# facebookresearch/seamless_communication

Hardware: AMD Instinct MI355X
Metric: S2ST utterances/sec (and real-time factor), seamlessM4T_v2_large, 10 s audio (higher is better)
Workload: dtype f32 activations x f16 weights, f32 accumulate

## Files before the change

### include/seamless_hip_internal.h

```cpp
#ifndef SEAMLESS_HIP_INTERNAL_H_
#define SEAMLESS_HIP_INTERNAL_H_

#include "seamless_hip.h"

#ifdef __cplusplus
extern "C" {
#endif

int sc_decoder_step_family(sc_model* m, int rows, int caller);

int sc_op_knob(const char* name, int dflt);

int sc_op_force_general_gemm(int on);
int32_t sc_op_voc_pack_plan(const int32_t* h_need, int32_t n, int64_t budget_rows, int32_t* h_group_first, int32_t cap);
int32_t sc_op_voc_tile_first(const int32_t* h_off, int32_t n, int32_t mul, int32_t tile_rows, int32_t* h_first);
int32_t sc_op_last_vocoder_packed_groups(sc_model* m);
int sc_op_single_plane(int on);
int sc_op_layernorm(const float* d_x, const float* d_gamma, const float* d_beta, float* d_y, int32_t rows, int32_t C,
                    int32_t act);
int sc_op_linear(const float* d_x, const void* d_w_f16, const float* d_bias, const float* d_res, float* d_y,
                 int32_t M, int32_t N, int32_t K, int32_t act, float alpha, int32_t split, int32_t force_gemv);
int sc_op_skinny_linear(const float* d_x, const void* d_w_f16, const float* d_bias, const float* d_res, float* d_y,
                        int32_t M, int32_t N, int32_t K, int32_t act, float alpha);
int sc_op_skinny_res_ln(const float* d_in, const void* d_w_f16, const float* d_bias, float* d_x_inout,
                        const float* d_gamma, const float* d_beta, float* d_h, int32_t M, int32_t N, int32_t K,
                        int32_t splits);
int sc_op_skinny_argmax(const float* d_x, const void* d_w_f16, int32_t M, int32_t N, int32_t K, int32_t step,
                        int32_t min_step_for_eos, int32_t force_eos_step, int32_t pad_idx, int32_t eos_idx,
                        int32_t unk_idx, float unk_penalty, int32_t* d_idx, float* d_lprob);

int sc_op_dstep_res_ln(const float* d_in, const void* d_w_f16, const float* d_bias, float* d_x_inout, const float* d_gamma,
                       const float* d_beta, float* d_h, int32_t M, int32_t N, int32_t K, int32_t splits);
int sc_op_dstep_linear_planes(const float* d_x, const void* d_w_f16, const float* d_bias, float* d_y, int32_t M, int32_t N, int32_t K,
                              int32_t act);
int sc_op_dstep_argmax(const float* d_x, const void* d_w_f16, int32_t M, int32_t N, int32_t K, int32_t step,
                       int32_t min_step_for_eos, int32_t force_eos_step, int32_t pad_idx, int32_t eos_idx, int32_t unk_idx,
                       float unk_penalty, int32_t ntl, int32_t* d_idx, float* d_lprob);
int sc_op_dstep_attention(const float* d_proj, int32_t S, const float* d_bias, float* d_kcache, float* d_vcache, int32_t cap,
                          int32_t pos, const int32_t* d_lens, int32_t cross, int32_t nb, int32_t heads, float* d_out);
int sc_op_dstep3_gemv(int32_t mode, const float* d_x, const void* d_w_f16, const float* d_bias, const float* d_gamma,
                      const float* d_beta, const float* d_res, float* d_y, float* d_h, int32_t M, int32_t N, int32_t K, int32_t act,
                      int32_t rg, int32_t shape);
int sc_op_dstep3_argmax(const float* d_x, const void* d_w_f16, int32_t M, int32_t N, int32_t K, int32_t step,
                        int32_t min_step_for_eos, int32_t force_eos_step, int32_t pad_idx, int32_t eos_idx, int32_t unk_idx,
                        float unk_penalty, int32_t* d_idx, float* d_lprob);
int sc_op_chain_bench(int32_t kind, int32_t rows, int32_t n, int32_t reps, float* us_per_kernel);
int sc_op_conv1d(const float* d_x, const void* d_w_f16_packed, const float* d_bias, const float* d_res, float* d_y,
                 int32_t nb, int32_t t_in, int32_t cin, int32_t cout, int32_t k, int32_t stride, int32_t pad,
                 int32_t dil, const int32_t* d_in_lens, int32_t in_act, int32_t act);
int sc_op_pack_conv_weight(const void* d_w_f16, void* d_dst_f16, int32_t cout, int32_t cin, int32_t k);
int sc_op_conv_transpose1d(const float* d_x, const void* d_v_f16, const void* d_g_f16, const float* d_bias,
                           float* d_y, int32_t nb, int32_t t_in, int32_t cin, int32_t cout, int32_t k,
                           int32_t stride, int32_t pad, int32_t in_act);
int sc_op_linear_presplit(const float* d_x, const void* d_w_f16, const float* d_bias, const float* d_res, float* d_y,
                          void* d_yh_f16, void* d_yl_f16, int32_t M, int32_t N, int32_t K, int32_t act, float alpha);
int sc_op_linear_presplit_argmax(const float* d_x, const void* d_w_f16, const float* d_bias, int32_t* d_idx, int32_t M, int32_t N,
                                 int32_t K);
int sc_op_conv1d_presplit(const float* d_x, const void* d_w_f16_packed, const float* d_bias, const float* d_res, float* d_y,
                          void* d_yh_f16, void* d_yl_f16, int32_t nb, int32_t t, int32_t cin, int32_t cout, int32_t k, int32_t pad,
                          int32_t dil, const unsigned char* d_row_valid, int32_t act);
int sc_op_resblock_pair_ps(const float* d_x, const void* d_w1_packed, const float* d_b1, const void* d_w2_packed, const float* d_b2,
                           float* d_out, int32_t nb, int32_t T, int32_t C, int32_t k, int32_t dil);
int sc_op_resblock_pair(const float* d_x, const void* d_w1_packed, const float* d_b1, const void* d_w2_packed,
                        const float* d_b2, float* d_out, int32_t nb, int32_t T, int32_t C, int32_t k, int32_t dil,
                        float slope, const float* d_avg_a, const float* d_avg_b);
int sc_op_mrf_fused(const float* d_x, const void* const* d_w1_packed, const float* const* d_b1, const void* const* d_w2_packed,
                    const float* const* d_b2, float* d_out, int32_t nb, int32_t T, int32_t C, const int32_t* k, const int32_t* dil,
                    float slope);
int sc_op_attention(const float* d_q, const float* d_k, const float* d_v, float* d_out, int32_t nb, int32_t heads,
                    int32_t sq, int32_t skv, int64_t ldq, int64_t ldk, int64_t ldv, int64_t ldo,
                    const int32_t* d_kv_lens, int32_t causal, const float* d_rel_k, int32_t rel_left,
                    int32_t rel_right);
int sc_op_attention_ex(const float* d_q, const float* d_k, const float* d_v, float* d_out, int32_t nb, int32_t heads,
                       int32_t sq, int32_t skv, int64_t ldq, int64_t ldk, int64_t ldv, int64_t ldo,
                       const int32_t* d_kv_lens, int32_t causal, const float* d_rel_k, int32_t rel_left,
                       int32_t rel_right, const int32_t* d_row_off, const float* d_rp_table, int64_t rp_ld,
                       const float* d_q_bias_u, const float* d_q_bias_v, void* d_out_hi, void* d_out_lo, int64_t ldoh);
int sc_op_glu_dwconv(const float* d_x, const float* d_w, float* d_y, int32_t nb, int32_t T, int32_t C, int32_t k,
                     const int32_t* d_lens);
int sc_op_glu_dwconv_ln(const float* d_x, const float* d_w, const float* d_gamma, const float* d_beta, int32_t act, void* d_yh_f16,
                        void* d_yl_f16, int32_t nb, int32_t T, int32_t C, int32_t k, const int32_t* d_lens, int32_t fused);
int sc_op_layernorm2(const float* d_x, const float* d_ga, const float* d_ba, const float* d_gb, const float* d_bb, float* d_y,
                     void* d_yh_f16, void* d_yl_f16, int32_t rows, int32_t C, int32_t fused);
int sc_op_argmax(const float* d_logits, int32_t rows, int32_t V, int32_t* d_idx, float* d_lprob);

int sc_op_beam_candidates(float* d_logits, int64_t ld, int32_t n_utt, int32_t beams, int32_t V, const float* d_cum, int32_t first_step,
                          int32_t no_eos, int32_t force_eos, int32_t pad_idx, int32_t eos_idx, int32_t unk_idx, float unk_penalty, int32_t K,
                          float* d_cand_val, int32_t* d_cand_idx, const int32_t* d_seqs, int32_t seq_ld, int32_t S, int32_t G,
                          const int32_t* d_rows, const int32_t* d_slots, int32_t chunked);
int sc_op_beam_candidates_banned(float* d_logits, int64_t ld, int32_t n_utt, int32_t beams, int32_t V, const float* d_cum,
                                 int32_t first_step, int32_t no_eos, int32_t force_eos, int32_t pad_idx, int32_t eos_idx, int32_t unk_idx,
                                 float unk_penalty, int32_t K, float* d_cand_val, int32_t* d_cand_idx, const int32_t* d_seqs,
                                 int32_t seq_ld, int32_t S, int32_t G, const int32_t* d_rows, const int32_t* d_slots, int32_t chunked,
                                 const int32_t* d_banned_tokens, const int32_t* d_banned_offsets, int32_t n_banned);
int sc_op_beam_select(const float* d_cand_val, const int32_t* d_cand_idx, const int32_t* d_seqs_cur, int32_t* d_seqs_new, float* d_fin_score,
                      int32_t* d_fin_len, int32_t* d_fin_seq, int32_t* d_fin_count, int32_t* d_done, int32_t* d_remaining, int32_t* d_tok,
                      int32_t* d_src_row, float* d_cum, int32_t* d_anc, int32_t anc_ld, const int32_t* d_slot_utt, const int32_t* d_slots,
                      int32_t n, int32_t beams, int32_t K, int32_t V, int32_t max_len, int32_t step, int32_t eos_idx, int32_t pad_idx,
                      int32_t normalize, float len_penalty);
int sc_op_beam_compact(const int32_t* d_done, int32_t* d_slot_utt, int32_t* d_slots, int32_t* d_rows, int32_t* d_seqs, float* d_cum,
                       int32_t* d_tok, int32_t* d_enc_lens, int32_t* d_anc, int32_t n, int32_t beams, int32_t max_len, int32_t anc_ld,
                       int32_t seq_len, int32_t anc_len);
int sc_op_gather_cache(const float* d_src, float* d_dst, const int32_t* d_src_row, int32_t rows, int32_t len, int32_t cap, int32_t M,
                       int32_t layers, int64_t layer_stride);
int sc_op_row_token_lprob(const float* d_logits, int64_t ld, int32_t rows, int32_t V, int32_t row_stride, int32_t token, float* d_out);

int sc_op_dstep_attention_ex(const float* d_proj, int32_t S, const float* d_bias, float* d_kcache, float* d_vcache, int32_t cap,
                             int32_t cache_rows, int32_t pos, const int32_t* d_lens, int32_t cross, int32_t nb, int32_t heads,
                             const int32_t* d_slot_rp, const int32_t* d_slot_lane, const int32_t* d_anc, const int32_t* d_kv_item,
                             int32_t kv_row_div, const int32_t* d_rows, float* d_out);
int sc_op_engine_step_close(const float* d_x, const void* d_w_f16, int32_t M, int32_t N, int32_t K, int32_t min_step_for_eos, int32_t pad_idx,
                            int32_t eos_idx, int32_t unk_idx, float unk_penalty, int32_t* d_slot_rp, const int32_t* d_rows, int32_t n_states,
                            int32_t cap, int32_t* d_tok, int32_t* d_pos, int32_t* d_finished, int32_t* d_out_len, const int32_t* d_limit,
                            const int32_t* d_prefix_len, float* d_score, int32_t* d_hist);
int sc_op_engine_admit(const int32_t* d_recs, int32_t n, int32_t n_states, int32_t cap, int32_t pad_idx, int32_t* d_tok, int32_t* d_pos,
                       int32_t* d_finished, int32_t* d_out_len, int32_t* d_limit, int32_t* d_prefix_len, int32_t* d_enc_lens, float* d_score,
                       int32_t* d_hist);
int sc_op_engine_set_slots(const int32_t* d_rids, int32_t n_live, int32_t slots, int32_t n_states, int32_t* d_slot_rp, int32_t* d_slot_lane,
                           const int32_t* d_pos, int32_t* d_rows);
int sc_op_engine_retire(const int32_t* h_rid, const int32_t* h_dst_rows, float* const* h_dst, int32_t n, int32_t n_states, int32_t cap, int32_t M,
                        const int32_t* d_out_len, const float* d_score, const int32_t* d_hist, const float* d_hidden, int32_t* d_stage);
int sc_op_dstep3_embed_ex(const int32_t* d_tok, const void* d_embed_f16, float scale, const float* d_pos_table, int32_t pos,
                          const int32_t* d_slot_rp, const int32_t* d_rows, int32_t rows, int32_t C, int32_t n_states, int32_t n_pos, int32_t vocab,
                          float* d_x);
int sc_op_dstep3_reduce_capture_ex(const float* d_partial, int32_t S, const float* d_bias, float* d_x_inout, const float* d_gamma, const float* d_beta,
                                   float* d_h, float* d_hrow, int64_t hrow_bs, int32_t hrow_rows, int32_t pos, const int32_t* d_slot_rp,
                                   const int32_t* d_rows, int32_t rows, int32_t C, int32_t n_states);
int sc_op_step_update(int32_t* d_next_tok, int32_t* d_hist, int32_t hist_ld, int32_t* d_finished, int32_t* d_out_len, const float* d_lprob,
                      float* d_score, int32_t nb, int32_t pos, int32_t pad_idx, int32_t eos_idx, int32_t* d_n_unfinished);
int sc_op_row_swap(float* d_k, float* d_v, float* d_cross, int32_t layers, int32_t pairs, const int32_t* h_src, const int32_t* h_dst, int32_t n_rows,
                   int32_t M, int32_t cap, int32_t s_enc, int32_t filled, int32_t* d_tok, int32_t* d_finished, int32_t* d_out_len,
                   int32_t* d_enc_lens, float* d_lprob, float* d_score, int32_t* d_hist, float* d_hidden);
int sc_op_align_lprob(const float* d_text, const float* d_feat, int32_t n, int32_t s_text, int32_t s_feat, int32_t C,
                      const int32_t* h_text_lens, const int32_t* h_feat_lens, float temperature, float* d_lprob);
int sc_op_mas(const float* d_lprob, int32_t n, int32_t s_text, int32_t s_feat, const int32_t* h_text_lens, const int32_t* h_feat_lens,
              int32_t* h_durations);
int sc_op_attention_hd(const float* d_q, const float* d_k, const float* d_v, float* d_out, int32_t nb, int32_t heads, int32_t sq, int32_t skv,
                       int64_t ldq, int64_t ldk, int64_t ldv, int64_t ldo, const int32_t* d_kv_lens, int32_t head_dim);
int sc_op_w2v2_frontend(const float* d_wav, int64_t wav_stride, const int32_t* h_num_samples, int32_t nb, const float* d_w, const float* d_bias,
                        const float* d_gamma, const float* d_beta, int32_t C, int32_t k, int32_t stride, float* d_out, int32_t t_rows,
                        float* d_stats);
int sc_op_w2v2_pos_conv(const float* d_x, const float* d_w, const float* d_bias, float* d_y, int32_t nb, int32_t T, int32_t C, int32_t groups,
                        int32_t k, const int32_t* d_lens);
int sc_op_kmeans(const float* d_x, const float* d_centroids, int32_t rows, int32_t C, int32_t K, int32_t* d_idx);

int sc_op_ecapa_chain(const float* d_x, const void* d_w_f16, const float* d_bias, const float* d_gamma, const float* d_beta, float* d_out, int32_t nb,
                      int32_t T, int32_t chunk, int32_t scale, int32_t dil);
int32_t sc_op_ecapa_chain_tile(int32_t chunk, int32_t scale, int32_t dil);
int sc_op_ecapa_relu_ln(const float* d_x, const float* d_item_bias, int32_t t_per_item, const float* d_gamma, const float* d_beta, float* d_y,
                        int32_t rows, int32_t C, int32_t act);
int sc_op_ecapa_se_gate(const float* d_x, int32_t nb, int32_t T, const int32_t* h_lens, int32_t C, int32_t S, const void* d_w1_f16, const float* d_b1,
                        const void* d_w2_f16, const float* d_b2, float* d_gate);
int sc_op_ecapa_pool(const float* d_x, const float* d_logits, int32_t nb, int32_t T, int32_t C, const int32_t* h_lens, float* d_pooled, float* d_gstats);
int sc_op_ecapa_tail(const float* d_pooled, int32_t nb, int32_t C2, const float* d_gamma, const float* d_beta, const void* d_w_f16, const float* d_bias,
                     int32_t E, float* d_out);
int32_t sc_op_prosody_last_launches(sc_prosody_encoder* p);

#ifdef __cplusplus
}
#endif
#endif
```

### seamless_communication_amd/_lib.py

```python
from __future__ import annotations

import ctypes as C
from pathlib import Path
from typing import Optional

import os

_VARIANT = os.environ.get("SC_LIB_VARIANT", "")
LIB_PATH = Path(__file__).resolve().parent / (f"libseamless_hip.{_VARIANT}.so" if _VARIANT else "libseamless_hip.so")

SC_ABI_VERSION = 10
SC_MAX_UPSAMPLES = 8
SC_MAX_RESBLOCK_KERNELS = 4
SC_MAX_RESBLOCK_DILATIONS = 4
SC_F16, SC_F32, SC_I32 = 0, 1, 2


class SeamlessHipError(RuntimeError):
    pass


class sc_tensor_desc(C.Structure):
    _fields_ = [
        ("name", C.c_char_p),
# ... 93 lines not shown
    "sc_abi_version": (C.c_int, []),
    "sc_load": (_P, [C.POINTER(sc_tensor_desc), C.c_size_t, C.POINTER(sc_config), C.c_int]),
    "sc_fork": (_P, [_P]),
    "sc_free": (None, [_P]),
    "sc_synchronize": (C.c_int, [_P]),
    "sc_wait_stream": (C.c_int, [_P, _P]),
    "sc_decoder_step_family": (C.c_int, [_P, C.c_int, C.c_int]),
    "sc_set_nar_tables": (C.c_int, [_P, _i, _P, _P, _P, _P, _P]),
    "sc_fbank": (C.c_int, [_P, _P, _i, C.c_int64, _P, _i, _P, _i, _P]),
    "sc_fbank_rate": (C.c_int, [_P, _P, _i, C.c_int64, _P, _i, _i, _P, _i, _P]),
    "sc_fbank_frames": (_i, [C.c_int64, _i]),
    "sc_encoder_out_len": (_i, [_P, _i]),
    "sc_encode_speech": (C.c_int, [_P, _P, _i, _i, _P, _P, _P]),
    "sc_encode_text": (C.c_int, [_P, _P, C.c_int32, C.c_int32, _P, _P]),
    "sc_mma_begin": (C.c_int, [_P, _P, C.c_int32, C.c_int32]),
    "sc_mma_step": (C.c_int, [_P, _P, C.c_int32, _P, C.c_int32, _P, _P, _P]),
    "sc_text_max_len": (_i, [_P, C.POINTER(sc_gen_opts), _i]),
    "sc_generate_text": (C.c_int, [_P, _P, _i, _i, _P, C.POINTER(sc_gen_opts), _P, _i, _P, _P, _P, _P]),
    "sc_generate_text_banned": (C.c_int, [_P, _P, _i, _i, _P, C.POINTER(sc_gen_opts), _P, _i, _P, _P, _P, _P, _P, _P, _i]),
    "sc_generate_text_capture": (C.c_int, [_P, _P, _i, _i, _P, C.POINTER(sc_gen_opts), _P, _i, _P, _P, _P, _P, _P, _P]),
    "sc_decode_text": (C.c_int, [_P, _P, _i, _i, _P, _P, _i, _P]),
    "sc_engine_create": (_P, [_P, C.POINTER(sc_engine_opts)]),
    "sc_engine_free": (None, [_P]),
    "sc_engine_attach": (C.c_int, [_P, _P]),
    "sc_engine_expect": (C.c_int, [_P, _i]),
    "sc_engine_get_stats": (C.c_int, [_P, C.POINTER(sc_engine_stats), _i]),
    "sc_t2u_nar": (C.c_int, [_P, _P, _i, _i, _P, _P, C.c_float, _P, _PI, _PI]),
    "sc_get_units": (C.c_int, [_P, _P]),
    "sc_get_durations": (C.c_int, [_P, _P, _P, _P]),
    "sc_vocoder_hop": (_i, [_P]),
    "sc_vocode": (C.c_int, [_P, _P, _i, _i, _P, _P, _P]),
    "sc_vocode_ragged": (C.c_int, [_P, _P, _i, _i, _P, _P, _P, _P]),
    "sc_vocoder_durations": (C.c_int, [_P, _P, _i, _i, _P]),
    "sc_t2u_ar": (C.c_int, [_P, _P, _i, _i, _P, C.POINTER(sc_gen_opts), _P, _i, _P, _i, _P, _P]),
    "sc_t2u_ar_max_len": (_i, [_P, C.POINTER(sc_gen_opts), _i]),
    "sc_last_padding": (C.c_int, [_P, _P, _P, _P]),
    "sc_s2st": (C.c_int, [_P, _P, _i, _i, _P, C.POINTER(sc_gen_opts), _P, _i, C.c_float, _P, _P, _P, _i, _P, _P, _i, _P, _P, _P]),
    "sc_prof_enable": (C.c_int, [C.c_int]),
    "sc_prof_reset": (C.c_int, []),
    "sc_prof_report": (C.c_int64, [C.c_char_p, C.c_int64]),
    "sc_text_to_char_seqs": (C.c_int32, [C.c_int32, _P, _P, _P, _P, _P, C.c_int32, C.c_int32, C.c_int32, _P, C.c_int32, C.c_int32,
                                         _P, _P, C.c_int32, _P]),
    "sc_ngram_blocked_tokens": (C.c_int32, [_PI, C.c_int32, C.c_int32, _PI, C.c_int32]),
    "sc_banned_blocked_tokens": (C.c_int32, [_PI, C.c_int32, _PI, _PI, C.c_int32, _PI, C.c_int32]),
    "sc_aligner_load": (_P, [C.POINTER(sc_tensor_desc), C.c_size_t, C.POINTER(sc_aligner_config), C.c_int]),
    "sc_aligner_free": (None, [_P]),
    "sc_align": (C.c_int, [_P, _P, _i, _i, _P, _P, _i, _P, _P, _P]),
    "sc_op_align_lprob": (C.c_int, [_P, _P, _i, _i, _i, _i, _P, _P, C.c_float, _P]),
    "sc_op_mas": (C.c_int, [_P, _i, _i, _i, _P, _P, _P]),
    "sc_unit_extractor_load": (_P, [C.POINTER(sc_tensor_desc), C.c_size_t, C.POINTER(sc_unit_extractor_config), C.c_int]),
    "sc_unit_extractor_free": (None, [_P]),
    "sc_unit_extractor_num_frames": (C.c_int32, [C.POINTER(sc_unit_extractor_config), C.c_int64]),
    "sc_extract_units": (C.c_int, [_P, _P, _i, C.c_int64, _P, _i, _P, _i, _P, _P]),
    "sc_op_attention_hd": (C.c_int, [_P, _P, _P, _P, _i, _i, _i, _i, C.c_int64, C.c_int64, C.c_int64, C.c_int64, _P, _i]),
    "sc_op_w2v2_frontend": (C.c_int, [_P, C.c_int64, _P, _i, _P, _P, _P, _P, _i, _i, _i, _P, _i, _P]),
    "sc_op_w2v2_pos_conv": (C.c_int, [_P, _P, _P, _P, _i, _i, _i, _i, _i, _P]),
    "sc_op_kmeans": (C.c_int, [_P, _P, _i, _i, _i, _P]),
    "sc_prosody_encoder_load": (_P, [C.POINTER(sc_tensor_desc), C.c_size_t, C.POINTER(sc_prosody_encoder_config), C.c_int]),
    "sc_prosody_encoder_free": (None, [_P]),
    "sc_prosody_encode": (C.c_int, [_P, _P, _i, _i, _P, _P, _P, _P]),
    "sc_op_ecapa_chain": (C.c_int, [_P, _P, _P, _P, _P, _P, _i, _i, _i, _i, _i]),
    "sc_op_ecapa_chain_tile": (C.c_int32, [_i, _i, _i]),
    "sc_op_ecapa_relu_ln": (C.c_int, [_P, _P, _i, _P, _P, _P, _i, _i, _i]),
    "sc_op_ecapa_se_gate": (C.c_int, [_P, _i, _i, _P, _i, _i, _P, _P, _P, _P, _P]),
    "sc_op_ecapa_pool": (C.c_int, [_P, _P, _i, _i, _i, _P, _P, _P]),
    "sc_op_ecapa_tail": (C.c_int, [_P, _i, _i, _P, _P, _P, _P, _i, _P]),
    "sc_op_prosody_last_launches": (C.c_int32, [_P]),
    "sc_op_knob": (C.c_int, [C.c_char_p, C.c_int]),
    "sc_op_force_general_gemm": (C.c_int, [C.c_int]),
    "sc_op_voc_pack_plan": (C.c_int32, [_PI, C.c_int32, C.c_int64, _PI, C.c_int32]),
    "sc_op_voc_tile_first": (C.c_int32, [_PI, C.c_int32, C.c_int32, C.c_int32, _PI]),
    "sc_op_last_vocoder_packed_groups": (C.c_int32, [_P]),
    "sc_op_single_plane": (C.c_int, [C.c_int]),
    "sc_op_layernorm": (C.c_int, [_P, _P, _P, _P, _i, _i, _i]),
    "sc_op_linear": (C.c_int, [_P, _P, _P, _P, _P, _i, _i, _i, _i, C.c_float, _i, _i]),
    "sc_op_skinny_linear": (C.c_int, [_P, _P, _P, _P, _P, _i, _i, _i, _i, C.c_float]),
    "sc_op_skinny_res_ln": (C.c_int, [_P, _P, _P, _P, _P, _P, _P, _i, _i, _i, _i]),
    "sc_op_skinny_argmax": (C.c_int, [_P, _P, _i, _i, _i, _i, _i, _i, _i, _i, _i, C.c_float, _P, _P]),
    "sc_op_dstep_res_ln": (C.c_int, [_P, _P, _P, _P, _P, _P, _P, _i, _i, _i, _i]),
    "sc_op_dstep_linear_planes": (C.c_int, [_P, _P, _P, _P, _i, _i, _i, _i]),
    "sc_op_dstep_argmax": (C.c_int, [_P, _P, _i, _i, _i, _i, _i, _i, _i, _i, _i, C.c_float, _i, _P, _P]),
    "sc_op_resblock_pair_ps": (C.c_int, [_P, _P, _P, _P, _P, _P, _i, _i, _i, _i, _i]),
    "sc_op_glu_dwconv_ln": (C.c_int, [_P, _P, _P, _P, _i, _P, _P, _i, _i, _i, _i, _P, _i]),
    "sc_op_layernorm2": (C.c_int, [_P, _P, _P, _P, _P, _P, _P, _P, _i, _i, _i]),
    "sc_op_dstep3_gemv": (C.c_int, [_i, _P, _P, _P, _P, _P, _P, _P, _P, _i, _i, _i, _i, _i, _i]),
    "sc_op_dstep3_argmax": (C.c_int, [_P, _P, _i, _i, _i, _i, _i, _i, _i, _i, _i, C.c_float, _P, _P]),
    "sc_op_chain_bench": (C.c_int, [_i, _i, _i, _i, _P]),
    "sc_op_dstep_attention": (C.c_int, [_P, _i, _P, _P, _P, _i, _i, _P, _i, _i, _i, _P]),
    "sc_op_conv1d": (C.c_int, [_P, _P, _P, _P, _P, _i, _i, _i, _i, _i, _i, _i, _i, _P, _i, _i]),
    "sc_op_pack_conv_weight": (C.c_int, [_P, _P, _i, _i, _i]),
    "sc_op_conv_transpose1d": (C.c_int, [_P, _P, _P, _P, _P, _i, _i, _i, _i, _i, _i, _i, _i]),
    "sc_op_linear_presplit": (C.c_int, [_P, _P, _P, _P, _P, _P, _P, _i, _i, _i, _i, C.c_float]),
    "sc_op_linear_presplit_argmax": (C.c_int, [_P, _P, _P, _P, _i, _i, _i]),
    "sc_op_conv1d_presplit": (C.c_int, [_P, _P, _P, _P, _P, _P, _P, _i, _i, _i, _i, _i, _i, _i, _P, _i]),
    "sc_op_mrf_fused": (C.c_int, [_P, _P, _P, _P, _P, _P, _i, _i, _i, _P, _P, C.c_float]),
    "sc_op_resblock_pair": (C.c_int, [_P, _P, _P, _P, _P, _P, _i, _i, _i, _i, _i, C.c_float, _P, _P]),
    "sc_op_attention": (C.c_int, [_P, _P, _P, _P, _i, _i, _i, _i, C.c_int64, C.c_int64, C.c_int64, C.c_int64, _P, _i,
                                  _P, _i, _i]),
    "sc_op_attention_ex": (C.c_int, [_P, _P, _P, _P, _i, _i, _i, _i, C.c_int64, C.c_int64, C.c_int64, C.c_int64, _P, _i,
                                     _P, _i, _i, _P, _P, C.c_int64, _P, _P, _P, _P, C.c_int64]),
    "sc_op_glu_dwconv": (C.c_int, [_P, _P, _P, _i, _i, _i, _i, _P]),
    "sc_op_argmax": (C.c_int, [_P, _i, _i, _P, _P]),
    "sc_op_beam_candidates": (C.c_int, [_P, C.c_int64, _i, _i, _i, _P, _i, _i, _i, _i, _i, _i, C.c_float, _i, _P, _P, _P, _i, _i, _i,
                                        _P, _P, _i]),
    "sc_op_beam_candidates_banned": (C.c_int, [_P, C.c_int64, _i, _i, _i, _P, _i, _i, _i, _i, _i, _i, C.c_float, _i, _P, _P, _P, _i, _i,
                                               _i, _P, _P, _i, _P, _P, _i]),
    "sc_op_beam_select": (C.c_int, [_P, _P, _P, _P, _P, _P, _P, _P, _P, _P, _P, _P, _P, _P, _i, _P, _P, _i, _i, _i, _i, _i, _i, _i, _i,
                                    _i, C.c_float]),
    "sc_op_beam_compact": (C.c_int, [_P, _P, _P, _P, _P, _P, _P, _P, _P, _i, _i, _i, _i, _i, _i]),
    "sc_op_gather_cache": (C.c_int, [_P, _P, _P, _i, _i, _i, _i, _i, C.c_int64]),
    "sc_op_row_token_lprob": (C.c_int, [_P, C.c_int64, _i, _i, _i, _i, _P]),
    "sc_op_dstep_attention_ex": (C.c_int, [_P, _i, _P, _P, _P, _i, _i, _i, _P, _i, _i, _i, _P, _P, _P, _P, _i, _P, _P]),
    "sc_op_engine_step_close": (C.c_int, [_P, _P, _i, _i, _i, _i, _i, _i, _i, C.c_float, _P, _P, _i, _i, _P, _P, _P, _P, _P, _P, _P, _P]),
    "sc_op_engine_admit": (C.c_int, [_P, _i, _i, _i, _i, _P, _P, _P, _P, _P, _P, _P, _P, _P]),
    "sc_op_engine_set_slots": (C.c_int, [_P, _i, _i, _i, _P, _P, _P, _P]),
    "sc_op_engine_retire": (C.c_int, [_P, _P, _P, _i, _i, _i, _i, _P, _P, _P, _P, _P]),
    "sc_op_dstep3_embed_ex": (C.c_int, [_P, _P, C.c_float, _P, _i, _P, _P, _i, _i, _i, _i, _i, _P]),
    "sc_op_dstep3_reduce_capture_ex": (C.c_int, [_P, _i, _P, _P, _P, _P, _P, _P, C.c_int64, _i, _i, _P, _P, _i, _i, _i]),
    "sc_op_step_update": (C.c_int, [_P, _P, _i, _P, _P, _P, _P, _i, _i, _i, _i, _P]),
    "sc_op_row_swap": (C.c_int, [_P, _P, _P, _i, _i, _P, _P, _i, _i, _i, _i, _i, _P, _P, _P, _P, _P, _P, _P, _P]),
}

_lib: Optional[C.CDLL] = None


def load_library() -> C.CDLL:
    global _lib
    if _lib is not None:
        return _lib
    if not LIB_PATH.exists():
        raise SeamlessHipError(
            f"{LIB_PATH} is missing: build it with `python -m seamless_communication_amd.build` "
            "(there is no CPU fallback for the HIP path)"
        )
    lib = C.CDLL(str(LIB_PATH))
    for name, (res, args) in SIGNATURES.items():
        fn = getattr(lib, name)
        fn.restype = res
        fn.argtypes = args
    if lib.sc_abi_version() != SC_ABI_VERSION:
        raise SeamlessHipError(f"ABI mismatch: library {lib.sc_abi_version()} vs binding {SC_ABI_VERSION}")
    _lib = lib
    return lib


def banned_csr(banned_seqs):
    import numpy as np

    seqs = [[int(t) for t in (s.tolist() if hasattr(s, "tolist") else s)] for s in banned_seqs]
    if any(len(s) == 0 for s in seqs):
        raise ValueError("a banned sequence must hold at least one token")
    off = np.zeros(len(seqs) + 1, dtype=np.int32)
    off[1:] = np.cumsum([len(s) for s in seqs], dtype=np.int64)
    tok = np.asarray([t for s in seqs for t in s], dtype=np.int32)
    return tok, off


def check(status: int, what: str) -> None:
    if status != 0:
        msg = load_library().sc_last_error()
        raise SeamlessHipError(f"{what} failed with status {status}: {msg.decode() if msg else '?'}")


def make_config(cfg, has_t2u: bool = True, has_vocoder: bool = True, has_text_encoder: bool = False,
                has_monotonic_decoder: bool = False, has_vocoder_dur_predictor: bool = False) -> sc_config:
    c = sc_config()
# ... 47 lines not shown
```

### seamless_communication_amd/csrc/api.hip

```cpp
#include <atomic>
#include <cstring>
#include <map>
#include <mutex>
#include <set>

#include "../../include/seamless_hip_internal.h"
#include "engine.h"
#include "model.h"

using namespace sc;

struct sc_model {
    Model m;
};

struct sc_engine {
    std::unique_ptr<Engine> e;
    int device = 0;
    const void* weights = nullptr;
    std::set<sc_model*> attached;
};

static std::mutex g_attach_mu;
static std::map<Engine*, sc_engine*> g_engine_owner;
// ... 1307 lines not shown
    a.out = d_out;
    a.ldq = ldq;
    a.ldk = ldk;
    a.ldv = ldv;
    a.ldo = ldo;
    a.nb = nb;
    a.heads = heads;
    a.Sq = sq;
    a.Skv = skv;
    a.kv_lens = d_kv_lens;
    a.causal = causal;
    a.rel_k = d_rel_k;
    a.rel_left = rel_left;
    a.rel_right = rel_right;
    launch_attention(a, g_op_stream);
    SC_HIP(hipStreamSynchronize(g_op_stream));
    SC_API_END
}

int sc_op_attention_ex(const float* d_q, const float* d_k, const float* d_v, float* d_out, int32_t nb, int32_t heads,
                       int32_t sq, int32_t skv, int64_t ldq, int64_t ldk, int64_t ldv, int64_t ldo, const int32_t* d_kv_lens,
                       int32_t causal, const float* d_rel_k, int32_t rel_left, int32_t rel_right, const int32_t* d_row_off,
                       const float* d_rp_table, int64_t rp_ld, const float* d_q_bias_u, const float* d_q_bias_v, void* d_out_hi,
                       void* d_out_lo, int64_t ldoh) {
    SC_API_BEGIN
    AttnArgs a;
    a.q = d_q;
    a.k = d_k;
    a.v = d_v;
    a.out = d_out;
    a.ldq = ldq;
    a.ldk = ldk;
    a.ldv = ldv;
    a.ldo = ldo;
    a.nb = nb;
    a.heads = heads;
    a.Sq = sq;
    a.Skv = skv;
    a.kv_lens = d_kv_lens;
    a.causal = causal;
    a.rel_k = d_rel_k;
    a.rel_left = rel_left;
    a.rel_right = rel_right;
    a.row_off = d_row_off;
    a.rp_table = d_rp_table;
    a.rp_ld = rp_ld;
    a.q_bias_u = d_q_bias_u;
    a.q_bias_v = d_q_bias_v;
    a.out_hi = static_cast<__half*>(d_out_hi);
    a.out_lo = static_cast<__half*>(d_out_lo);
    a.ldoh = ldoh;
    launch_attention(a, g_op_stream);
    SC_HIP(hipStreamSynchronize(g_op_stream));
    SC_API_END
}

int sc_op_glu_dwconv(const float* d_x, const float* d_w, float* d_y, int32_t nb, int32_t T, int32_t C, int32_t k,
                     const int32_t* d_lens) {
    SC_API_BEGIN
    launch_glu_dwconv(d_x, 2 * C, d_w, d_y, C, nb, T, C, k, d_lens, g_op_stream);
    SC_HIP(hipStreamSynchronize(g_op_stream));
    SC_API_END
}

int sc_op_glu_dwconv_ln(const float* d_x, const float* d_w, const float* d_gamma, const float* d_beta, int32_t act, void* d_yh_f16,
                        void* d_yl_f16, int32_t nb, int32_t T, int32_t C, int32_t k, const int32_t* d_lens, int32_t fused) {
    SC_API_BEGIN
    SC_CHECK(d_x && d_w && d_gamma && d_beta && d_yh_f16 && d_yl_f16, "sc_op_glu_dwconv_ln: null argument");
    __half* yh = static_cast<__half*>(d_yh_f16);
    __half* yl = static_cast<__half*>(d_yl_f16);
    if (fused) {
        launch_glu_dwconv_ln(d_x, 2 * C, d_w, d_gamma, d_beta, act, yh, yl, C, nb, T, C, k, d_lens, g_op_stream);
    } else {
        OpScratch scratch;
        float* mid = scratch.get<float>((size_t)nb * T * C);
        launch_glu_dwconv(d_x, 2 * C, d_w, mid, C, nb, T, C, k, d_lens, g_op_stream);
        launch_layernorm_split(mid, C, d_gamma, d_beta, yh, yl, C, nb * T, C, act, nullptr, 1, g_op_stream);
        SC_HIP(hipStreamSynchronize(g_op_stream));
    }
    SC_HIP(hipStreamSynchronize(g_op_stream));
    SC_API_END
}

int sc_op_layernorm2(const float* d_x, const float* d_ga, const float* d_ba, const float* d_gb, const float* d_bb, float* d_y,
                     void* d_yh_f16, void* d_yl_f16, int32_t rows, int32_t C, int32_t fused) {
    SC_API_BEGIN
    SC_CHECK(d_x && d_ga && d_ba && d_gb && d_bb && d_y && d_yh_f16 && d_yl_f16, "sc_op_layernorm2: null argument");
    __half* yh = static_cast<__half*>(d_yh_f16);
    __half* yl = static_cast<__half*>(d_yl_f16);
    if (fused) {
        launch_layernorm2_split(d_x, C, d_ga, d_ba, d_y, C, d_gb, d_bb, yh, yl, C, rows, C, g_op_stream);
    } else {
        launch_layernorm(d_x, C, d_ga, d_ba, d_y, C, rows, C, ACT_NONE, nullptr, 1, g_op_stream);
        launch_layernorm_split(d_y, C, d_gb, d_bb, yh, yl, C, rows, C, ACT_NONE, nullptr, 1, g_op_stream);
    }
    SC_HIP(hipStreamSynchronize(g_op_stream));
    SC_API_END
}

int sc_op_argmax(const float* d_logits, int32_t rows, int32_t V, int32_t* d_idx, float* d_lprob) {
    SC_API_BEGIN
    launch_argmax_rows(d_logits, V, rows, V, nullptr, -1, -1, -1, -1, -1, 0.f, d_idx, d_lprob, g_op_stream);
    SC_HIP(hipStreamSynchronize(g_op_stream));
    SC_API_END
}


static int op_beam_candidates(float* d_logits, int64_t ld, int32_t n_utt, int32_t beams, int32_t V, const float* d_cum, int32_t first_step,
                              int32_t no_eos, int32_t force_eos, int32_t pad_idx, int32_t eos_idx, int32_t unk_idx, float unk_penalty, int32_t K,
                              float* d_cand_val, int32_t* d_cand_idx, const int32_t* d_seqs, int32_t seq_ld, int32_t S, int32_t G,
                              const int32_t* d_rows, const int32_t* d_slots, int32_t chunked, const int32_t* d_banned_tokens,
                              const int32_t* d_banned_offsets, int32_t n_banned) {
    SC_API_BEGIN
    BannedList bl;
    if (n_banned != 0) {
        SC_CHECK(n_banned > 0 && n_banned <= BANNED_MAX_SEQS && d_banned_tokens && d_banned_offsets && d_seqs,
                 "sc_op_beam_candidates_banned: bad banned list (n_banned=%d; needs d_seqs)", n_banned);
        const std::vector<int32_t> off = op_read_ints(d_banned_offsets, (size_t)n_banned + 1);
        SC_CHECK(off[0] == 0 && off[n_banned] >= 0 && off[n_banned] <= BANNED_MAX_TOKENS, "sc_op_beam_candidates_banned: bad offsets");
        for (int q = 0; q < n_banned; ++q) SC_CHECK(off[q + 1] >= off[q], "sc_op_beam_candidates_banned: offsets decrease at %d", q);
        const std::vector<int32_t> tok = op_read_ints(d_banned_tokens, (size_t)off[n_banned]);
        validate_banned_host(tok.data(), off.data(), n_banned, V, &bl.max_len);
        bl.tokens = d_banned_tokens, bl.offsets = d_banned_offsets, bl.n = n_banned;
    }
    const BannedList* banned = bl.n > 0 ? &bl : nullptr;
    SC_CHECK(d_logits && d_cum && d_cand_val && d_cand_idx && n_utt >= 1 && V >= 1 && ld >= V, "sc_op_beam_candidates: bad arguments");
    SC_CHECK(!d_seqs || (G >= 0 && S >= 0 && seq_ld >= S), "sc_op_beam_candidates: bad n-gram arguments (S=%d G=%d seq_ld=%d)", S, G, seq_ld);
    if (d_slots) SC_CHECK(op_read_ints(d_slots, 1)[0] <= n_utt, "sc_op_beam_candidates: *d_slots > n_utt");
    if (chunked) {
        SC_CHECK(beam_chunked(V, beams, K), "sc_op_beam_candidates: the chunked search does not take V=%d beams=%d K=%d", V, beams, K);
        if (d_rows) SC_CHECK(op_read_ints(d_rows, 1)[0] <= n_utt * beams, "sc_op_beam_candidates: *d_rows > n_utt * beams");
        OpScratch scratch;
        const int rows = n_utt * beams;
        float* ws_f = scratch.get<float>(beam_ws_floats(rows, K));
        int* ws_i = scratch.get<int>(beam_ws_ints(rows, K));
        SC_HIP(hipMemsetAsync(ws_f, 0xff, beam_ws_floats(rows, K) * 4, g_op_stream));
        SC_HIP(hipMemsetAsync(ws_i, 0xff, beam_ws_ints(rows, K) * 4, g_op_stream));
        launch_beam_candidates_chunked(d_logits, ld, n_utt, beams, V, d_cum, first_step, no_eos, force_eos, pad_idx, eos_idx, unk_idx,
                                       unk_penalty, K, d_cand_val, d_cand_idx, d_seqs, seq_ld, S, G, ws_f, ws_i, g_op_stream, d_rows, d_slots, banned);
        SC_HIP(hipStreamSynchronize(g_op_stream));
    } else {
        SC_CHECK(!d_rows, "sc_op_beam_candidates: d_rows is an argument of the chunked search only (the single-workgroup one takes d_slots)");
        launch_beam_candidates(d_logits, ld, n_utt, beams, V, d_cum, first_step, no_eos, force_eos, pad_idx, eos_idx, unk_idx, unk_penalty, K,
                               d_cand_val, d_cand_idx, d_seqs, seq_ld, S, G, g_op_stream, d_slots, banned);
        SC_HIP(hipStreamSynchronize(g_op_stream));
    }
    SC_API_END
}

int sc_op_beam_candidates(float* d_logits, int64_t ld, int32_t n_utt, int32_t beams, int32_t V, const float* d_cum, int32_t first_step,
                          int32_t no_eos, int32_t force_eos, int32_t pad_idx, int32_t eos_idx, int32_t unk_idx, float unk_penalty, int32_t K,
                          float* d_cand_val, int32_t* d_cand_idx, const int32_t* d_seqs, int32_t seq_ld, int32_t S, int32_t G,
                          const int32_t* d_rows, const int32_t* d_slots, int32_t chunked) {
    return op_beam_candidates(d_logits, ld, n_utt, beams, V, d_cum, first_step, no_eos, force_eos, pad_idx, eos_idx, unk_idx, unk_penalty, K,
                              d_cand_val, d_cand_idx, d_seqs, seq_ld, S, G, d_rows, d_slots, chunked, nullptr, nullptr, 0);
}

int sc_op_beam_candidates_banned(float* d_logits, int64_t ld, int32_t n_utt, int32_t beams, int32_t V, const float* d_cum,
                                 int32_t first_step, int32_t no_eos, int32_t force_eos, int32_t pad_idx, int32_t eos_idx, int32_t unk_idx,
                                 float unk_penalty, int32_t K, float* d_cand_val, int32_t* d_cand_idx, const int32_t* d_seqs,
                                 int32_t seq_ld, int32_t S, int32_t G, const int32_t* d_rows, const int32_t* d_slots, int32_t chunked,
                                 const int32_t* d_banned_tokens, const int32_t* d_banned_offsets, int32_t n_banned) {
    return op_beam_candidates(d_logits, ld, n_utt, beams, V, d_cum, first_step, no_eos, force_eos, pad_idx, eos_idx, unk_idx, unk_penalty, K,
                              d_cand_val, d_cand_idx, d_seqs, seq_ld, S, G, d_rows, d_slots, chunked, d_banned_tokens, d_banned_offsets,
                              n_banned);
}
// ... 349 lines not shown
```

### seamless_communication_amd/csrc/common.cpp

```cpp
#include "common.h"
#include <cstdlib>
#include <cstring>

namespace sc {

static thread_local char g_err[1024] = "";

void set_error(const char* fmt, ...) {
    va_list ap;
    va_start(ap, fmt);
    vsnprintf(g_err, sizeof(g_err), fmt, ap);
    va_end(ap);
}

const char* get_error() { return g_err; }

namespace knob {
namespace {
struct Knob {
    const char* name;
    int kind;
    const char* what;
};
const Knob knob_table[] = {
    {"SC_DEBUG_NUMERICS", 0, "honour the switches that change results"},
    {"SC_DEBUG_FILL", 0, "fill fresh scratch blocks with NaN (tests)"},
    {"SC_SPLIT_MODE", 1, "1: Conformer products on the hi fp16 plane only (precision study)"},
    {"SC_DECODER_GEN1", 1, "decoder step on the first-generation kernels"},
    {"SC_DECODER_GEN2", 1, "decoder step on the second-generation chain"},
    {"SC_DECODE_STEPWISE", 1, "teacher-forced pass step by step instead of one batched forward"},
    {"SC_VOC_SPLIT", 1, "vocoder ResBlock products on both fp16 planes of their activations again (bit 0 wide stages, bit 2 narrow stages); default: hi plane only"},
    {"SC_GEMM_GENERAL", 0, "general GEMM kernel instead of the fast path"}, {"SC_GEMM_PF2", 0, "GEMM prefetch depth"},
    {"SC_GEMM_GROUP_M", 0, "GEMM workgroup order"}, {"SC_GEMM_TILE", 0, "GEMM tile override"},
    {"SC_PS_TILE", 0, "DMA GEMM: largest tile"}, {"SC_PS_MIN256", 0, "DMA GEMM: tiles needed for 256 x 256"},
    {"SC_PS_MIN128", 0, "DMA GEMM: tiles needed for 128 x 128"},
    {"SC_PRESPLIT", 0, "0: Conformer operands split on the fly"}, {"SC_ENC_FUSE", 0, "0: separate Conformer element-wise launches"},
    {"SC_D3_RG_SMALL", 0, "decoder step: rows per row group, N = 1024 products"}, {"SC_D3_RG_FFN", 0, "decoder step: rows per row group, FFN-in"},
    {"SC_G3_STATIONARY", 0, "row-group products of wide steps: 0 one workgroup per row group, n = workgroup budget of the weight-stationary launch"},
    {"SC_G3_TILES", 0, "0: FFN-out of wide steps on the weight-stationary row-group walk instead of tile-owning waves"},
    {"SC_G3_TOUCH", 0, "weight-stationary products: bit 0 cooperative L2 touch of the activations, bit 1 K slices per XCD (FFN-out); default 3"},
    {"SC_D3_FFN_IN", 0, "decoder step: FFN-in workgroup shape"}, {"SC_D3_FFN_OUT", 0, "decoder step: FFN-out workgroup shape"},
    {"SC_T2U_GROUPS", 0, "NAR T2U: length buckets"}, {"SC_T2U_PACKED", 0, "0: NAR decoder on padded buckets"},
    {"SC_VOC_PS", 0, "0: vocoder wide stages on the register-staged convolution"}, {"SC_VOC_MRF", 0, "0: narrow vocoder stages as nine pair launches"},
    {"SC_VOC_GROUPS", 0, "vocoder: length buckets"}, {"SC_VOC_GROUP_OVERHEAD", 0, "vocoder: bucket planning overhead rows"},
    {"SC_VOC_STREAMS", 0, "vocoder: side chains"},
    {"SC_VOC_PACKED", 0, "0: ragged vocoder batches in length buckets on side chains instead of the packed pass"},
    {"SC_VOC_PACK_ROWS", 0, "vocoder: unit rows per packed group"},
    {"SC_ENGINE_RG_SMALL", 0, "decode engine: rows per row group, N = 1024 products"},
    {"SC_BEAM_COMPACT", 2, "0: beam search keeps finished utterances' slots"},
    {"SC_GREEDY_COMPACT", 2, "0: greedy generation keeps finished rows in their slots"}, {"SC_GREEDY_POLL", 2, "steps between looks at the finished flags"},
};
constexpr int N_KNOBS = sizeof(knob_table) / sizeof(knob_table[0]);
struct State {
    bool set[N_KNOBS];
    int val[N_KNOBS];
    bool numerics = false;
};
const State& state() {
    static const State st = [] {
        State s{};
        const char* dn = getenv("SC_DEBUG_NUMERICS");
        s.numerics = dn && atoi(dn) != 0;
        for (int i = 0; i < N_KNOBS; ++i) {
            const char* e = getenv(knob_table[i].name);
            s.set[i] = e != nullptr && (knob_table[i].kind != 1 || s.numerics);
            s.val[i] = e ? atoi(e) : 0;
        }
        return s;
    }();
    return st;
}
int lookup(const char* name) {
    for (int i = 0; i < N_KNOBS; ++i)
        if (strcmp(knob_table[i].name, name) == 0) return i;
    return -1;
}
int find(const char* name) {
    const int i = lookup(name);
    if (i >= 0) return i;
    fprintf(stderr, "libseamless_hip: switch %s is not in the knob table (common.cpp)\n", name);
    abort();
}
}

bool known(const char* name) { return name && lookup(name) >= 0; }

int value(const char* name, int dflt) {
    const int i = find(name);
    return state().set[i] ? state().val[i] : dflt;
}
bool is_set(const char* name) { return state().set[find(name)]; }
int live(const char* name, int dflt) {
    (void)find(name);
    const char* e = getenv(name);
    return e ? atoi(e) : dflt;
}
void report_once() {
    static const bool done = [] {
        const State& s = state();
        for (int i = 0; i < N_KNOBS; ++i) {
            const char* e = getenv(knob_table[i].name);
            if (!e || knob_table[i].kind == 2) continue;
            if (knob_table[i].kind == 1 && !s.numerics)
                fprintf(stderr, "libseamless_hip: %s=%s IGNORED - it changes results (%s); set SC_DEBUG_NUMERICS=1 to honour it\n", knob_table[i].name, e,
                        knob_table[i].what);
            else
                fprintf(stderr, "libseamless_hip: %s=%s (%s)%s\n", knob_table[i].name, e, knob_table[i].what, knob_table[i].kind == 1 ? " - RESULTS CHANGE" : "");
        }
        return true;
    }();
    (void)done;
}
}

}
```

### seamless_communication_amd/csrc/k_gemm_ps.hip

```cpp
#include <cstdlib>
#include <type_traits>

#include "kernels.h"

namespace sc {

typedef _Float16 half8_t __attribute__((ext_vector_type(8)));
typedef float float16_t __attribute__((ext_vector_type(16)));

namespace {

constexpr int PBK = 32;
#define SC_LDS_PTR(p) ((__attribute__((address_space(3))) void*)(p))

template <int ACT>
__device__ __forceinline__ float ps_act(float v) {
    if (ACT == ACT_RELU) return v > 0.f ? v : 0.f;
    if (ACT == ACT_SILU) return v / (1.f + expf(-v));
    if (ACT == ACT_TANH) return tanhf(v);
    return v;
}

typedef int i32x4_t __attribute__((ext_vector_type(4)));

__device__ __forceinline__ i32x4_t make_rsrc_words(const void* base, uint32_t bytes) {
    const uint64_t b = reinterpret_cast<uint64_t>(base);
    i32x4_t r;
    r[0] = __builtin_amdgcn_readfirstlane((int)(uint32_t)b);
    r[1] = __builtin_amdgcn_readfirstlane((int)(uint32_t)((b >> 32) & 0xffff));
    r[2] = __builtin_amdgcn_readfirstlane((int)bytes);
    r[3] = 0x00020000;
    return r;
}

__device__ __forceinline__ int swz(int row, int s) { return row * 64 + ((s ^ ((row >> 2) & 3)) << 4); }

template <int WM, int WN, int EP_LD, int ACT>
__device__ __forceinline__ void ps_epilogue(const GemmPsArgs& p, const float* ep, int m0w, int n0w, int lane) {
    typedef float f4_t __attribute__((ext_vector_type(4)));
    typedef _Float16 h4_t __attribute__((ext_vector_type(4)));
    constexpr int LPR = WN / 4;
    constexpr int RPG = 16 / LPR;
    constexpr int RPI = 4 * RPG;
    const int l5 = lane & 31;
    const bool g1 = (l5 >= 4 && l5 < 12) || (l5 >= 16 && l5 < 20) || l5 >= 28;
    const int rank = g1 ? (l5 < 12 ? l5 - 4 : l5 < 20 ? l5 - 8 : l5 - 16) : (l5 < 4 ? l5 : l5 < 16 ? l5 - 8 : l5 - 12);
    const int grp = (lane >> 5) * 2 + (g1 ? 1 : 0);
    const int row_in = grp * RPG + rank / LPR;
    const int c0 = (rank % LPR) * 4;
    const int col = n0w + c0;
    const bool vec_ok = (col + 3 < p.N) && ((p.ldc | p.ldr | p.ldcs) % 4 == 0) && (n0w % 4 == 0);
    f4_t b4 = {0.f, 0.f, 0.f, 0.f};
    if (p.bias) {
#pragma unroll
        for (int e = 0; e < 4; ++e) b4[e] = (col + e < p.N) ? p.bias[col + e] : 0.f;
    }
#pragma unroll
    for (int it = 0; it < WM / RPI; ++it) {
        const int row = it * RPI + row_in;
        const int64_t m = m0w + row;
        const f4_t a = *reinterpret_cast<const f4_t*>(ep + row * EP_LD + c0);
        if (m >= p.M || col >= p.N) continue;
        const bool dead = p.row_valid && p.row_valid[m] == 0;
        f4_t v;
#pragma unroll
        for (int e = 0; e < 4; ++e) v[e] = dead ? 0.f : ps_act<ACT>(a[e] + b4[e]) * p.alpha;
        if (vec_ok) {
            if (p.res && !dead) v += *reinterpret_cast<const f4_t*>(p.res + m * p.ldr + col);
            if (p.C) *reinterpret_cast<f4_t*>(p.C + m * p.ldc + col) = v;
            if (p.Ch) {
                if (p.plane_neg_slope != 1.0f) {
#pragma unroll
                    for (int e = 0; e < 4; ++e) v[e] = fmaxf(v[e], 0.f) + p.plane_neg_slope * fminf(v[e], 0.f);
                }
                const h4_t hi = __builtin_convertvector(v, h4_t);
                *reinterpret_cast<h4_t*>(reinterpret_cast<_Float16*>(p.Ch) + m * p.ldcs + col) = hi;
                if (p.Cl)
                    *reinterpret_cast<h4_t*>(reinterpret_cast<_Float16*>(p.Cl) + m * p.ldcs + col) =
                        __builtin_convertvector(v - __builtin_convertvector(hi, f4_t), h4_t);
            }
        } else {
#pragma unroll
            for (int e = 0; e < 4; ++e) {
                if (col + e >= p.N) continue;
                float x = v[e];
                if (p.res && !dead) x += p.res[m * p.ldr + col + e];
                if (p.C) p.C[m * p.ldc + col + e] = x;
                if (p.Ch) {
                    if (p.plane_neg_slope != 1.0f) x = fmaxf(x, 0.f) + p.plane_neg_slope * fminf(x, 0.f);
                    const _Float16 h = (_Float16)x;
                    reinterpret_cast<_Float16*>(p.Ch)[m * p.ldcs + col + e] = h;
                    if (p.Cl) reinterpret_cast<_Float16*>(p.Cl)[m * p.ldcs + col + e] = (_Float16)(x - (float)h);
                }
            }
        }
    }
}

template <int BM, int BN, int WGM, int WGN, bool SPLIT, bool CONV, bool AMAX>
__global__ __launch_bounds__(WGM* WGN * 64) void gemm_ps_kernel(GemmPsArgs p, int tiles_n, int tiles_total, int tiles_per_xcd,
                                                                 uint32_t a_bytes, uint32_t w_bytes) {
    constexpr int NWAVE = WGM * WGN;
    constexpr bool ALTERNATE = SPLIT && NWAVE == 8;
    constexpr bool MID_BARRIER = SPLIT && !ALTERNATE;
    constexpr int WM = BM / WGM, WN = BN / WGN;
    constexpr int TM = WM / 32, TN = WN / 32;
    constexpr int ACH = BM / (16 * NWAVE);
    constexpr int BCH = BN / (16 * NWAVE);
    constexpr uint32_t OOB = 0x80000000u;
    constexpr int A_TILE = BM * 32, B_TILE = BN * 32;

    constexpr int A_PL = SPLIT ? 2 : 1;
    constexpr int STAGE_BYTES = (A_PL * A_TILE + B_TILE) * 2;
    constexpr int EPN = WN < 64 ? WN : (NWAVE * WM * (64 + 4) * 4 <= 3 * STAGE_BYTES ? 64 : 32);
    constexpr int EP_LD = EPN + 4;
    static_assert(NWAVE * WM * EP_LD * 4 <= 3 * STAGE_BYTES, "epilogue tiles must fit in the stage memory");
    __shared__ __attribute__((aligned(16))) char smem[3 * STAGE_BYTES];
    _Float16* const sAh0 = reinterpret_cast<_Float16*>(smem);
    _Float16* const sAl0 = sAh0 + (A_PL - 1) * A_TILE;
    _Float16* const sB0 = sAh0 + A_PL * A_TILE;
    _Float16* const sAh1 = reinterpret_cast<_Float16*>(smem + STAGE_BYTES);
    _Float16* const sAl1 = sAh1 + (A_PL - 1) * A_TILE;
    _Float16* const sB1 = sAh1 + A_PL * A_TILE;
    _Float16* const sAh2 = reinterpret_cast<_Float16*>(smem + 2 * STAGE_BYTES);
    _Float16* const sAl2 = sAh2 + (A_PL - 1) * A_TILE;
    _Float16* const sB2 = sAh2 + A_PL * A_TILE;

    const int bid = blockIdx.x;
    const int tile = (bid & 7) * tiles_per_xcd + (bid >> 3);
    if (tile >= tiles_total) return;
    const int tm = tile / tiles_n;
    const int tn = tile - tm * tiles_n;
    const int tid = threadIdx.x, lane = tid & 63, wave = tid >> 6;
    const int wm = wave / WGN, wn = wave % WGN;
    const int m0 = tm * BM, n0 = tn * BN;

    const i32x4_t rah = make_rsrc_words(p.Ah, a_bytes);
    const i32x4_t ral = make_rsrc_words(p.Al, a_bytes);
    const i32x4_t rw = make_rsrc_words(p.W, w_bytes);

    uint32_t a_voff[ACH], b_voff[BCH];
    int a_t[ACH];
    int a_len[ACH];
#pragma unroll
    for (int j = 0; j < ACH; ++j) {
        const int row = 16 * (wave * ACH + j) + (lane >> 2);
        const int seg = (lane & 3) ^ ((row >> 2) & 3);
        a_voff[j] = (m0 + row) < p.M ? (uint32_t)(((int64_t)(m0 + row) * p.lda + seg * 8) * 2) : OOB;
        a_t[j] = 0;
        a_len[j] = 0;
        if (CONV) {
            if (p.row_pos) {
                const int2 rp = (m0 + row) < p.M ? p.row_pos[m0 + row] : make_int2(0, 0);
                a_t[j] = rp.x;
                a_len[j] = rp.y;
            } else {
                a_t[j] = (m0 + row) % p.rows_per_item;
                a_len[j] = p.rows_per_item;
            }
        }
    }
    int nx_tap = 0, nx_cs = 0, nx_slab = 0;
    const int spt = CONV ? p.conv_cin / PBK : 1;
    const uint32_t row_bytes = (uint32_t)(p.lda * 2);
    uint32_t va_[ACH];
    int ka_ = 0;
#define PS_NEXT_ADDR()                                                                                  \
    do {                                                                                                \
        if (CONV) {                                                                                     \
            const int dt_ = nx_tap * p.conv_dil - p.conv_pad;                                           \
            ka_ = nx_cs * (PBK * 2);                                                                    \
            _Pragma("unroll") for (int j = 0; j < ACH; ++j) {                                           \
                const bool in_ = (uint32_t)(a_t[j] + dt_) < (uint32_t)a_len[j] && a_voff[j] != OOB;     \
                va_[j] = in_ ? a_voff[j] + (uint32_t)dt_ * row_bytes : OOB;                             \
            }                                                                                           \
            if (++nx_cs == spt) {                                                                       \
                nx_cs = 0;                                                                              \
                ++nx_tap;                                                                               \
            }                                                                                           \
        } else {                                                                                        \
            ka_ = nx_slab * (PBK * 2);                                                                  \
            _Pragma("unroll") for (int j = 0; j < ACH; ++j) va_[j] = a_voff[j];                         \
        }                                                                                               \
        ++nx_slab;                                                                                      \
// ... 189 lines not shown
        _Pragma("unroll") for (int i = 0; i < TM; ++i)                                                                 \
            _Pragma("unroll") for (int j = 0; j < TN; ++j) {                                                           \
                acc[i][j] = __builtin_amdgcn_mfma_f32_32x32x16_f16(c_ah[i], c_bf[j], acc[i][j], 0, 0, 0);               \
                acc[i][j] = __builtin_amdgcn_mfma_f32_32x32x16_f16(c_al[i], c_bf[j], acc[i][j], 0, 0, 0);               \
                if (q_ < NDMA) {                                                                                       \
                    __builtin_amdgcn_sched_barrier(0);                                                                 \
                    if (iss2_) PS_DMA_Q(q_, OAH, OAL, OB, ((S) + 2) * (PBK * 2));                                      \
                    __builtin_amdgcn_sched_barrier(0);                                                                 \
                }                                                                                                      \
                ++q_;                                                                                                  \
            }                                                                                                          \
        _Pragma("unroll") for (int q2 = NH + TM * TN; q2 < NDMA; ++q2)                                                 \
            if (iss2_) PS_DMA_Q(q2, OAH, OAL, OB, ((S) + 2) * (PBK * 2));                                              \
        if ((S) + 1 < nslab) {                                                                                         \
            if (iss2_) __builtin_amdgcn_s_waitcnt(NDMA == 6 ? 0x0076 : 0x0073);           \
            else __builtin_amdgcn_s_waitcnt(0x0070);                                          \
            __builtin_amdgcn_s_barrier();                                                                              \
            asm volatile("" ::: "memory");                                                                             \
            PS_READ_C0(NAH, NAL, NB);                                                                                  \
        }                                                                                                              \
        const bool iss3_ = (S) + 3 < nslab;                                                                            \
        if (iss3_) PS_NEXT_ADDR();                                                                                     \
        __builtin_amdgcn_sched_barrier(0);                                                                             \
        q_ = 0;                                                                                                        \
        _Pragma("unroll") for (int i = 0; i < TM; ++i)                                                                 \
            _Pragma("unroll") for (int j = 0; j < TN; ++j) {                                                           \
                acc[i][j] = __builtin_amdgcn_mfma_f32_32x32x16_f16(ah1[i], bf1[j], acc[i][j], 0, 0, 0);                 \
                acc[i][j] = __builtin_amdgcn_mfma_f32_32x32x16_f16(al1[i], bf1[j], acc[i][j], 0, 0, 0);                 \
                if (q_ < NH) {                                                                                         \
                    __builtin_amdgcn_sched_barrier(0);                                                                 \
                    if (iss3_) PS_DMA_Q(q_, CAH, CAL, CB, ((S) + 3) * (PBK * 2));                                      \
                    __builtin_amdgcn_sched_barrier(0);                                                                 \
                }                                                                                                      \
                ++q_;                                                                                                  \
            }                                                                                                          \
        asm volatile("" ::: "memory");                                                                                 \
    } while (0)

        PS_ISSUE(sAh0, sAl0, sB0, 0);
        if (nslab > 1) PS_ISSUE(sAh1, sAl1, sB1, PBK * 2);
        if (nslab > 2) {
            PS_NEXT_ADDR();
#pragma unroll
            for (int q = 0; q < NH; ++q) PS_DMA_Q(q, sAh2, sAl2, sB2, 2 * (PBK * 2));
        }
        if (nslab > 2) __builtin_amdgcn_s_waitcnt(NDMA == 6 ? 0x0079 : 0x0074);
        else if (nslab > 1) __builtin_amdgcn_s_waitcnt(NDMA == 6 ? 0x0076 : 0x0073);
        else __builtin_amdgcn_s_waitcnt(0x0070);
        __builtin_amdgcn_s_barrier();
        asm volatile("" ::: "memory");
        PS_READ_C0(sAh0, sAl0, sB0);
        for (int s = 0; s < nslab; s += 3) {
            PS_HSTEP(s, sAh0, sAl0, sB0, sAh1, sAl1, sB1, sAh2, sAl2, sB2);
            if (s + 1 < nslab) PS_HSTEP(s + 1, sAh1, sAl1, sB1, sAh2, sAl2, sB2, sAh0, sAl0, sB0);
            if (s + 2 < nslab) PS_HSTEP(s + 2, sAh2, sAl2, sB2, sAh0, sAl0, sB0, sAh1, sAl1, sB1);
        }
#undef PS_HSTEP
#undef PS_READ_C0
    } else {
        PS_ISSUE(sAh0, sAl0, sB0, 0);
        if (nslab > 1) PS_ISSUE(sAh1, sAl1, sB1, PBK * 2);
        for (int s = 0; s < nslab; s += 3) {
            PS_STEP(s, sAh0, sB0, sAh2, sB2);
            if (s + 1 < nslab) PS_STEP(s + 1, sAh1, sB1, sAh0, sB0);
            if (s + 2 < nslab) PS_STEP(s + 2, sAh2, sB2, sAh1, sB1);
        }
    }
#undef PS_STEP
#undef PS_LDS8
#undef PS_DMA_Q
#undef PS_NEXT_ADDR
#undef PS_ISSUE
#undef PS_DMA

    __builtin_amdgcn_s_waitcnt(0x0070);
    __builtin_amdgcn_s_barrier();
    asm volatile("" ::: "memory");
    float* ep = reinterpret_cast<float*>(smem) + wave * (WM * EP_LD);
    const int m0w = m0 + wm * WM;
    float am_best = -INFINITY;
    int am_idx = 0x7fffffff;
    auto pass = [&](auto hc) {
        constexpr int h = decltype(hc)::value;
#pragma unroll
        for (int i = 0; i < TM; ++i)
#pragma unroll
            for (int j = 0; j < EPN / 32; ++j)
#pragma unroll
                for (int r = 0; r < 16; ++r)
                    ep[(i * 32 + (r & 3) + 8 * (r >> 2) + 4 * (lane >> 5)) * EP_LD + j * 32 + (lane & 31)] = acc[i][h * (EPN / 32) + j][r];
        const int n0w = n0 + wn * WN + h * EPN;
        if constexpr (AMAX) {
            typedef float f4_t __attribute__((ext_vector_type(4)));
            if (lane < WM) {
                const float* row = ep + lane * EP_LD;
#pragma unroll
                for (int c4 = 0; c4 < EPN / 4; ++c4) {
                    const f4_t a = *reinterpret_cast<const f4_t*>(row + 4 * c4);
#pragma unroll
                    for (int e = 0; e < 4; ++e) {
                        const int col = n0w + 4 * c4 + e;
                        if (col < p.N) {
                            const float v = (a[e] + (p.bias ? p.bias[col] : 0.f)) * p.alpha;
                            if (v > am_best) {
                                am_best = v;
                                am_idx = col;
                            }
                        }
                    }
                }
            }
            return;
        }
        if (p.act == ACT_NONE) ps_epilogue<WM, EPN, EP_LD, ACT_NONE>(p, ep, m0w, n0w, lane);
        else if (p.act == ACT_RELU) ps_epilogue<WM, EPN, EP_LD, ACT_RELU>(p, ep, m0w, n0w, lane);
        else if (p.act == ACT_SILU) ps_epilogue<WM, EPN, EP_LD, ACT_SILU>(p, ep, m0w, n0w, lane);
        else ps_epilogue<WM, EPN, EP_LD, ACT_TANH>(p, ep, m0w, n0w, lane);
    };
    static_assert(WN % EPN == 0 && WN / EPN >= 1 && WN / EPN <= 4, "one to four epilogue passes");
    pass(std::integral_constant<int, 0>{});
    if constexpr (WN / EPN > 1) pass(std::integral_constant<int, 1>{});
    if constexpr (WN / EPN > 2) pass(std::integral_constant<int, 2>{});
    if constexpr (WN / EPN > 3) pass(std::integral_constant<int, 3>{});
    if constexpr (AMAX) {
        const int64_t m = m0w + lane;
        if (lane < WM && m < p.M) p.amax[m * p.amax_ld + tn * WGN + wn] = make_float2(am_best, __int_as_float(am_idx));
    }
}

template <int BM, int BN, int WGM, int WGN>
void launch_ps_cfg(const GemmPsArgs& a, hipStream_t s) {
    const int tiles_m = cdiv(a.M, BM), tiles_n = cdiv(a.N, BN);
    const int tiles_total = tiles_m * tiles_n;
    const int tiles_per_xcd = cdiv(tiles_total, 8);
    char name[64];
    snprintf(name, sizeof(name), "gemm_%dx%d_presplit", BM, BN);
    prof::Scope scope(name, 2.0 * a.M * (double)a.N * a.K,
                      4.0 * a.M * (double)a.K + 2.0 * a.N * (double)a.K + (a.amax ? 8.0 * a.M * (double)a.amax_ld : 4.0 * a.M * (double)a.N * (a.res ? 2.0 : 1.0)), s);
    const dim3 grid(tiles_per_xcd * 8), block(WGM * WGN * 64);
    const uint32_t ab = (uint32_t)((int64_t)a.M * a.lda * 2), wb = (uint32_t)((int64_t)a.N * a.ldw * 2);
    const auto launch = [&](auto kernel) { hipLaunchKernelGGL(kernel, grid, block, 0, s, a, tiles_n, tiles_total, tiles_per_xcd, ab, wb); };
    const bool conv = a.conv_taps > 0;
    if (a.amax) launch(gemm_ps_kernel<BM, BN, WGM, WGN, true, false, true>);
    else if (a.split && conv) launch(gemm_ps_kernel<BM, BN, WGM, WGN, true, true, false>);
    else if (a.split) launch(gemm_ps_kernel<BM, BN, WGM, WGN, true, false, false>);
    else if (conv) launch(gemm_ps_kernel<BM, BN, WGM, WGN, false, true, false>);
    else launch(gemm_ps_kernel<BM, BN, WGM, WGN, false, false, false>);
}

int ps_tile(int M, int N) {
    static const int max_tile = knob::value("SC_PS_TILE", 256);
    const int64_t tiles128 = (int64_t)cdiv(M, 128) * cdiv(N, 128);
    const int64_t tiles256 = (int64_t)cdiv(M, 256) * cdiv(N, 256);
    static const int min256 = knob::value("SC_PS_MIN256", 224);
    static const int min128 = knob::value("SC_PS_MIN128", 256);
    if (max_tile >= 256 && tiles256 >= min256 && N > 128) return 256;
    return tiles128 >= min128 ? 128 : 64;
}

}

void launch_gemm_presplit(const GemmPsArgs& a, hipStream_t s) {
    SC_CHECK(a.Ah && (a.Al || !a.split) && a.W && (a.C || a.Ch || a.amax), "presplit gemm: null operand");
    SC_CHECK(a.Ch || !a.Cl, "presplit gemm: a lo output plane needs its hi plane");
    SC_CHECK(a.act >= ACT_NONE && a.act <= ACT_TANH, "presplit gemm: activation %d has no epilogue here", a.act);
    SC_CHECK(a.M > 0 && a.N > 0 && a.K > 0 && a.K % PBK == 0, "presplit gemm: M=%d N=%d K=%d (K must be a multiple of 32)", a.M, a.N, a.K);
    SC_CHECK(a.lda % 8 == 0 && a.ldw % 8 == 0 && a.ldw >= a.K, "presplit gemm: lda=%lld ldw=%lld", (long long)a.lda,
             (long long)a.ldw);
    SC_CHECK(((reinterpret_cast<uintptr_t>(a.Ah) | reinterpret_cast<uintptr_t>(a.Al) | reinterpret_cast<uintptr_t>(a.W) |
               reinterpret_cast<uintptr_t>(a.C) | reinterpret_cast<uintptr_t>(a.res)) & 15) == 0 &&
                 ((reinterpret_cast<uintptr_t>(a.Ch) | reinterpret_cast<uintptr_t>(a.Cl)) & 7) == 0,
             "presplit gemm: operands must be 16-byte aligned");
    SC_CHECK((int64_t)a.M * a.lda * 2 < (1ll << 31) && (int64_t)a.N * a.ldw * 2 < (1ll << 31), "presplit gemm: operand larger than 2 GB");
    if (a.conv_taps > 0) {
        SC_CHECK(a.conv_cin % PBK == 0 && a.K == a.conv_taps * a.conv_cin && a.lda >= a.conv_cin &&
                     (a.row_pos || (a.rows_per_item > 0 && a.M % a.rows_per_item == 0)) && a.conv_dil >= 1 && a.conv_pad >= 0,
                 "presplit conv: taps=%d cin=%d K=%d rows_per_item=%d M=%d", a.conv_taps, a.conv_cin, a.K, a.rows_per_item, a.M);
    } else {
        SC_CHECK(a.lda >= a.K, "presplit gemm: lda=%lld < K=%d", (long long)a.lda, a.K);
    }
    if (a.amax) {
        SC_CHECK(a.split && a.conv_taps == 0 && !a.C && !a.Ch && !a.res && !a.row_valid && a.act == ACT_NONE,
                 "presplit gemm: the fused arg-max takes a plain product (no C / planes / residual / activation)");
        SC_CHECK(a.amax_ld == gemm_presplit_amax_chunks(a.M, a.N), "presplit gemm: amax_ld=%d, this shape produces %d partial results per row",
                 a.amax_ld, gemm_presplit_amax_chunks(a.M, a.N));
    }
    const int tile = ps_tile(a.M, a.N);
    if (tile == 256) launch_ps_cfg<256, 256, 4, 2>(a, s);
    else if (tile == 128) launch_ps_cfg<128, 128, 2, 2>(a, s);
    else launch_ps_cfg<64, 64, 2, 2>(a, s);
    SC_LAUNCH_CHECK();
}

int gemm_presplit_amax_chunks(int M, int N) { return 2 * cdiv(N, ps_tile(M, N)); }

namespace {
__global__ __launch_bounds__(256) void amax_finish_kernel(const float2* __restrict__ part, int ld, int rows, int* __restrict__ out_idx) {
    const int lane = threadIdx.x & 63;
    const int row = blockIdx.x * 4 + (threadIdx.x >> 6);
    if (row >= rows) return;
    const float2* pr = part + (int64_t)row * ld;
    float best = -INFINITY;
    int bidx = 0x7fffffff;
    for (int i = lane; i < ld; i += 64) {
        const float2 v = pr[i];
        const int vi = __float_as_int(v.y);
        if (v.x > best || (v.x == best && vi < bidx)) {
            best = v.x;
            bidx = vi;
        }
    }
#pragma unroll
    for (int o = 32; o > 0; o >>= 1) {
        const float ob = __shfl_xor(best, o);
        const int oi = __shfl_xor(bidx, o);
        if (ob > best || (ob == best && oi < bidx)) {
            best = ob;
            bidx = oi;
        }
    }
    if (lane == 0) out_idx[row] = bidx;
}
}

void launch_amax_finish(const float2* part, int ld, int rows, int* out_idx, hipStream_t s) {
    if (rows <= 0) return;
    hipLaunchKernelGGL(amax_finish_kernel, dim3(cdiv(rows, 4)), dim3(256), 0, s, part, ld, rows, out_idx);
    SC_LAUNCH_CHECK();
}

}
```

### seamless_communication_amd/csrc/k_misc.hip

```cpp
#include "kernels.h"

namespace sc {

__global__ __launch_bounds__(256) void embed_tokens_kernel(const int* __restrict__ tokens, int rows,
                                                           const __half* __restrict__ emb, int M,
                                                           float scale, const float* __restrict__ pos_table,
                                                           const int* __restrict__ d_pos, int t_per_batch,
                                                           float* __restrict__ out, int64_t ldo) {
    const int row = blockIdx.x;
    const int tok = tokens[row];
    const int pos = (d_pos ? *d_pos : 0) + (t_per_batch > 0 ? row % t_per_batch : 0);
    const __half* e = emb + (int64_t)tok * M;
    const float* pe = pos_table + (int64_t)pos * M;
    for (int c = threadIdx.x; c < M; c += 256) out[(int64_t)row * ldo + c] = __half2float(e[c]) * scale + pe[c];
}

void launch_embed_tokens(const int* tokens, int rows, const __half* emb, int M, float scale,
                         const float* pos_table, const int* d_pos, int t_per_batch, float* out, int64_t ldo,
                         hipStream_t s) {
    if (rows <= 0) return;
    hipLaunchKernelGGL(embed_tokens_kernel, dim3(rows), dim3(256), 0, s, tokens, rows, emb, M, scale, pos_table,
                       d_pos, t_per_batch, out, ldo);
    SC_LAUNCH_CHECK();
}
// ... 304 lines not shown
                                                        int rows, int H, int t_per_batch,
                                                        const int* __restrict__ lens, float duration_factor,
                                                        int min_dur, int* __restrict__ durations) {
    const int lane = threadIdx.x & 63;
    const int row = blockIdx.x * 4 + (threadIdx.x >> 6);
    if (row >= rows) return;
    const float* hr = h + (int64_t)row * ld;
    float acc = 0.f;
    for (int c = lane; c < H; c += 64) acc = fmaf(hr[c], w[c], acc);
#pragma unroll
    for (int o = 32; o > 0; o >>= 1) acc += __shfl_xor(acc, o);
    if (lane == 0) {
        const int n = row / t_per_batch, t = row - n * t_per_batch;
        int d = 0;
        if (!lens || t < lens[n]) {
            const float x = acc + b[0];
            const float r = rintf((expf(x) - 1.0f) * duration_factor);
            long long dl = (long long)r;
            if (dl < (long long)min_dur) dl = min_dur;
            if (dl > 1000000) dl = 1000000;
            d = (int)dl;
        }
        durations[row] = d;
    }
}
void launch_durations(const float* h, int64_t ld, const float* w, const float* b, int rows, int H, int t_per_batch,
                      const int* lens, float duration_factor, int min_dur, int* durations, hipStream_t s) {
    if (rows <= 0) return;
    hipLaunchKernelGGL(durations_kernel, dim3(cdiv(rows, 4)), dim3(256), 0, s, h, ld, w, b, rows, H, t_per_batch, lens,
                       duration_factor, min_dur, durations);
    SC_LAUNCH_CHECK();
}

__global__ __launch_bounds__(256) void vocoder_embed_kernel(const int* __restrict__ units, int T,
                                                            const __half* __restrict__ dict, int E,
                                                            const __half* __restrict__ lang, int Lg,
                                                            const int* __restrict__ lang_idx,
                                                            const __half* __restrict__ spkr, int Sp,
                                                            const int* __restrict__ spkr_idx,
                                                            float* __restrict__ out, const int* __restrict__ item_off, int n_items) {
    const int row = blockIdx.x;
    const int n = item_off ? item_search(n_items, row, [&](int i) { return item_off[i]; }) : row / T;
    const int C = Lg + E + Sp;
    const __half* l = lang + (int64_t)lang_idx[n] * Lg;
    const __half* d = dict + (int64_t)units[row] * E;
    const __half* sp = spkr + (int64_t)spkr_idx[n] * Sp;
    float* o = out + (int64_t)row * C;
    for (int c = threadIdx.x; c < C; c += 256) {
        __half v;
        if (c < Lg) v = l[c];
        else if (c < Lg + E) v = d[c - Lg];
        else v = sp[c - Lg - E];
        o[c] = __half2float(v);
    }
}
void launch_vocoder_embed(const int* units, int nb, int T, const __half* dict, int E, const __half* lang, int Lg,
                          const int* lang_idx, const __half* spkr, int Sp, const int* spkr_idx, float* out,
                          hipStream_t s, const int* item_off, int rows_total) {
    const int rows = item_off ? rows_total : nb * T;
    if (rows <= 0) return;
    hipLaunchKernelGGL(vocoder_embed_kernel, dim3(rows), dim3(256), 0, s, units, T, dict, E, lang, Lg, lang_idx, spkr,
                       Sp, spkr_idx, out, item_off, nb);
    SC_LAUNCH_CHECK();
}

__global__ void avg3_kernel(const float* __restrict__ a, const float* __restrict__ b, const float* __restrict__ c,
                            float* __restrict__ out, int64_t n) {
    for (int64_t i = (int64_t)blockIdx.x * blockDim.x + threadIdx.x; i < n; i += (int64_t)gridDim.x * blockDim.x)
        out[i] = ((a[i] + b[i]) + c[i]) / 3.0f;
}
__global__ void split_f32_kernel(const float* __restrict__ x, __half* __restrict__ hi, __half* __restrict__ lo, int64_t n4) {
    typedef _Float16 h4_t __attribute__((ext_vector_type(4)));
    typedef float f4_t __attribute__((ext_vector_type(4)));
    for (int64_t i = (int64_t)blockIdx.x * blockDim.x + threadIdx.x; i < n4; i += (int64_t)gridDim.x * blockDim.x) {
        const f4_t v = reinterpret_cast<const f4_t*>(x)[i];
        const h4_t h = __builtin_convertvector(v, h4_t);
        reinterpret_cast<h4_t*>(hi)[i] = h;
        reinterpret_cast<h4_t*>(lo)[i] = __builtin_convertvector(v - __builtin_convertvector(h, f4_t), h4_t);
    }
}
void launch_split_f32(const float* x, __half* hi, __half* lo, int64_t n, hipStream_t s) {
    SC_CHECK(n % 4 == 0, "split_f32: n must be a multiple of 4");
    if (n <= 0) return;
    hipLaunchKernelGGL(split_f32_kernel, dim3(grid_for(n / 4)), dim3(256), 0, s, x, hi, lo, n / 4);
    SC_LAUNCH_CHECK();
}

__global__ void lrelu_split_f32_kernel(const float* __restrict__ x, float neg_slope, __half* __restrict__ hi, __half* __restrict__ lo,
                                       int64_t n4) {
    typedef _Float16 h4_t __attribute__((ext_vector_type(4)));
    typedef float f4_t __attribute__((ext_vector_type(4)));
    for (int64_t i = (int64_t)blockIdx.x * blockDim.x + threadIdx.x; i < n4; i += (int64_t)gridDim.x * blockDim.x) {
        f4_t v = reinterpret_cast<const f4_t*>(x)[i];
#pragma unroll
        for (int e = 0; e < 4; ++e) v[e] = fmaxf(v[e], 0.f) + neg_slope * fminf(v[e], 0.f);
        const h4_t h = __builtin_convertvector(v, h4_t);
        reinterpret_cast<h4_t*>(hi)[i] = h;
        if (lo) reinterpret_cast<h4_t*>(lo)[i] = __builtin_convertvector(v - __builtin_convertvector(h, f4_t), h4_t);
    }
}
void launch_lrelu_split_f32(const float* x, float neg_slope, __half* hi, __half* lo, int64_t n, hipStream_t s) {
    SC_CHECK(n % 4 == 0, "lrelu_split_f32: n must be a multiple of 4");
    if (n <= 0) return;
    hipLaunchKernelGGL(lrelu_split_f32_kernel, dim3(grid_for(n / 4)), dim3(256), 0, s, x, neg_slope, hi, lo, n / 4);
    SC_LAUNCH_CHECK();
}

void launch_avg3(const float* a, const float* b, const float* c, float* out, int64_t n, hipStream_t s) {
    if (n <= 0) return;
    hipLaunchKernelGGL(avg3_kernel, dim3(grid_for(n)), dim3(256), 0, s, a, b, c, out, n);
    SC_LAUNCH_CHECK();
}

template <int C, int K>
__global__ __launch_bounds__(256) void conv_to_mono_kernel(const float* __restrict__ x, const __half* __restrict__ w, const float* __restrict__ bias,
                                                           float slope, int act, float* __restrict__ y, int T,
                                                           const int* __restrict__ item_off, int item_mul) {
    constexpr int RS = C + 4, ROWS = 256 + K - 1, VPR = C / 4;
    typedef float f4_t __attribute__((ext_vector_type(4)));
    __shared__ __attribute__((aligned(16))) float tile[ROWS * RS];
    __shared__ __attribute__((aligned(16))) float sw[K * C];
    const int tid = threadIdx.x, n = blockIdx.y;
    const int t0 = blockIdx.x * 256;
    int64_t row0 = (int64_t)n * T;
    if (item_off) {
        row0 = (int64_t)item_off[n] * item_mul;
        T = (item_off[n + 1] - item_off[n]) * item_mul;
        if (t0 >= T) return;
    }
    const float* __restrict__ xn = x + row0 * C;
    for (int i = tid; i < ROWS * VPR; i += 256) {
        const int r = i / VPR, c4 = i - r * VPR;
        const int t = t0 - K / 2 + r;
        f4_t v = {0.f, 0.f, 0.f, 0.f};
        if (t >= 0 && t < T) v = *reinterpret_cast<const f4_t*>(xn + (int64_t)t * C + c4 * 4);
#pragma unroll
        for (int j = 0; j < 4; ++j) v[j] = v[j] > 0.f ? v[j] : slope * v[j];
        *reinterpret_cast<f4_t*>(tile + r * RS + c4 * 4) = v;
    }
    for (int i = tid; i < K * C; i += 256) sw[i] = __half2float(w[i]);
    __syncthreads();
    const int t = t0 + tid;
    if (t >= T) return;
    float acc = 0.f;
#pragma unroll
    for (int tap = 0; tap < K; ++tap)
#pragma unroll
        for (int c4 = 0; c4 < VPR; ++c4) {
            const f4_t xv = *reinterpret_cast<const f4_t*>(tile + (tid + tap) * RS + c4 * 4);
            const f4_t wv = *reinterpret_cast<const f4_t*>(sw + tap * C + c4 * 4);
#pragma unroll
            for (int j = 0; j < 4; ++j) acc = fmaf(xv[j], wv[j], acc);
        }
    acc += bias ? bias[0] : 0.f;
    y[row0 + t] = act == ACT_TANH ? tanhf(acc) : acc;
}

bool conv_to_mono_supported(int cin, int cout, int k, int stride, int pad, int dil, int act) {
    return cout == 1 && cin == 16 && k == 7 && stride == 1 && dil == 1 && 2 * pad == k - 1 && (act == ACT_NONE || act == ACT_TANH);
}

void launch_conv_to_mono(const float* x, const __half* w_packed, const float* bias, int nb, int T, int cin, int k, float in_slope, int act,
                         float* y, hipStream_t s, const int* item_off, int item_mul, int64_t rows_total) {
    SC_CHECK(conv_to_mono_supported(cin, 1, k, 1, (k - 1) / 2, 1, act), "conv_to_mono: unsupported cin=%d k=%d act=%d", cin, k, act);
    if (nb <= 0 || T <= 0) return;
    const double rows = item_off ? (double)rows_total : nb * (double)T;
// ... 134 lines not shown
```

### seamless_communication_amd/csrc/k_norm.hip

```cpp
#include "kernels.h"

namespace sc {

__device__ __forceinline__ float wave_sum(float v) {
#pragma unroll
    for (int o = 32; o > 0; o >>= 1) v += __shfl_xor(v, o);
    return v;
}

__device__ __forceinline__ float act_f(float v, int act) {
    if (act == ACT_RELU) return v > 0.f ? v : 0.f;
    if (act == ACT_SILU) return v / (1.f + expf(-v));
    if (act == ACT_GELU) return 0.5f * v * (1.f + erff(v * 0.70710678118654752440f));
    return v;
}

template <int MAXV>
__global__ __launch_bounds__(256) void layernorm_kernel(const float* __restrict__ x, int64_t ldx,
                                                        const float* __restrict__ gamma,
                                                        const float* __restrict__ beta,
                                                        float* __restrict__ y, int64_t ldy, int rows,
                                                        int C, int act, const int* __restrict__ lens,
                                                        int t_per_batch, __half* __restrict__ yh = nullptr,
                                                        __half* __restrict__ yl = nullptr, int64_t ldh = 0) {
// ... 66 lines not shown
            }
            if (!yh || both) yr[idx] = o;
        }
    }
}

__global__ __launch_bounds__(256) void layernorm2_kernel(const float* __restrict__ x, int64_t ldx, const float* __restrict__ ga,
                                                         const float* __restrict__ ba, float* __restrict__ y, int64_t ldy,
                                                         const float* __restrict__ gb2, const float* __restrict__ bb2,
                                                         __half* __restrict__ yh, __half* __restrict__ yl, int64_t ldh, int rows, int C) {
    typedef _Float16 h4_t __attribute__((ext_vector_type(4)));
    typedef float f4_t __attribute__((ext_vector_type(4)));
    const int lane = threadIdx.x & 63;
    const int row = blockIdx.x * 4 + (threadIdx.x >> 6);
    if (row >= rows) return;
    const int nv = C >> 2;
    const float4* xr = reinterpret_cast<const float4*>(x + (int64_t)row * ldx);
    float4* yr = reinterpret_cast<float4*>(y + (int64_t)row * ldy);
    h4_t* yhr = reinterpret_cast<h4_t*>(yh + (int64_t)row * ldh);
    h4_t* ylr = reinterpret_cast<h4_t*>(yl + (int64_t)row * ldh);
    float4 v[4];
    float s = 0.f;
#pragma unroll
    for (int i = 0; i < 4; ++i) {
        const int idx = lane + 64 * i;
        v[i] = idx < nv ? xr[idx] : make_float4(0.f, 0.f, 0.f, 0.f);
        s += (v[i].x + v[i].y) + (v[i].z + v[i].w);
    }
    float mean = wave_sum(s) / (float)C;
    float q = 0.f;
#pragma unroll
    for (int i = 0; i < 4; ++i) {
        const int idx = lane + 64 * i;
        if (idx < nv) {
            const float a = v[i].x - mean, b = v[i].y - mean, c = v[i].z - mean, d = v[i].w - mean;
            q += (a * a + b * b) + (c * c + d * d);
        }
    }
    float rstd = 1.0f / sqrtf(wave_sum(q) / (float)C + 1e-5f);
    s = 0.f;
#pragma unroll
    for (int i = 0; i < 4; ++i) {
        const int idx = lane + 64 * i;
        if (idx < nv) {
            const float4 g = reinterpret_cast<const float4*>(ga)[idx], b = reinterpret_cast<const float4*>(ba)[idx];
            v[i].x = (v[i].x - mean) * rstd * g.x + b.x;
            v[i].y = (v[i].y - mean) * rstd * g.y + b.y;
            v[i].z = (v[i].z - mean) * rstd * g.z + b.z;
            v[i].w = (v[i].w - mean) * rstd * g.w + b.w;
            yr[idx] = v[i];
        }
        s += (v[i].x + v[i].y) + (v[i].z + v[i].w);
    }
    mean = wave_sum(s) / (float)C;
    q = 0.f;
#pragma unroll
    for (int i = 0; i < 4; ++i) {
        const int idx = lane + 64 * i;
        if (idx < nv) {
            const float a = v[i].x - mean, b = v[i].y - mean, c = v[i].z - mean, d = v[i].w - mean;
            q += (a * a + b * b) + (c * c + d * d);
        }
    }
    rstd = 1.0f / sqrtf(wave_sum(q) / (float)C + 1e-5f);
#pragma unroll
    for (int i = 0; i < 4; ++i) {
        const int idx = lane + 64 * i;
        if (idx < nv) {
            const float4 g = reinterpret_cast<const float4*>(gb2)[idx], b = reinterpret_cast<const float4*>(bb2)[idx];
            const f4_t of = {(v[i].x - mean) * rstd * g.x + b.x, (v[i].y - mean) * rstd * g.y + b.y, (v[i].z - mean) * rstd * g.z + b.z,
                             (v[i].w - mean) * rstd * g.w + b.w};
            const h4_t hi = __builtin_convertvector(of, h4_t);
            const f4_t back = __builtin_convertvector(hi, f4_t);
            yhr[idx] = hi;
            ylr[idx] = __builtin_convertvector(of - back, h4_t);
        }
    }
}

void launch_layernorm2_split(const float* x, int64_t ldx, const float* ga, const float* ba, float* y, int64_t ldy, const float* gb2,
                             const float* bb2, __half* yh, __half* yl, int64_t ldh, int rows, int C, hipStream_t s) {
    SC_CHECK(C % 4 == 0 && C <= 1024 && ldx % 4 == 0 && ldy % 4 == 0 && ldh % 4 == 0 && y && yh && yl, "layernorm2_split: C=%d", C);
    if (rows <= 0) return;
    hipLaunchKernelGGL(layernorm2_kernel, dim3(cdiv(rows, 4)), dim3(256), 0, s, x, ldx, ga, ba, y, ldy, gb2, bb2, yh, yl, ldh, rows, C);
    SC_LAUNCH_CHECK();
}

void launch_layernorm_split(const float* x, int64_t ldx, const float* gamma, const float* beta, __half* yh, __half* yl,
                            int64_t ldh, int rows, int C, int act, const int* lens, int t_per_batch, hipStream_t s) {
    SC_CHECK(C % 4 == 0 && ldx % 4 == 0 && ldh % 4 == 0 && C <= 4096 && yh && yl, "layernorm_split: C=%d ldx=%lld ldh=%lld", C,
             (long long)ldx, (long long)ldh);
    if (rows <= 0) return;
    dim3 grid(cdiv(rows, 4));
    float* none = nullptr;
    if (C <= 256) hipLaunchKernelGGL((layernorm_kernel<1>), grid, dim3(256), 0, s, x, ldx, gamma, beta, none, (int64_t)0, rows, C, act, lens, t_per_batch, yh, yl, ldh);
    else if (C <= 1024) hipLaunchKernelGGL((layernorm_kernel<4>), grid, dim3(256), 0, s, x, ldx, gamma, beta, none, (int64_t)0, rows, C, act, lens, t_per_batch, yh, yl, ldh);
    else hipLaunchKernelGGL((layernorm_kernel<16>), grid, dim3(256), 0, s, x, ldx, gamma, beta, none, (int64_t)0, rows, C, act, lens, t_per_batch, yh, yl, ldh);
    SC_LAUNCH_CHECK();
}

void launch_layernorm_both(const float* x, int64_t ldx, const float* gamma, const float* beta, float* y, int64_t ldy, __half* yh,
                           __half* yl, int64_t ldh, int rows, int C, int act, const int* lens, int t_per_batch, hipStream_t s) {
    SC_CHECK(C % 4 == 0 && ldx % 4 == 0 && ldy % 4 == 0 && ldh % 4 == 0 && C <= 4096 && y && yh && yl, "layernorm_both: C=%d", C);
    if (rows <= 0) return;
    dim3 grid(cdiv(rows, 4));
    if (C <= 256) hipLaunchKernelGGL((layernorm_kernel<1>), grid, dim3(256), 0, s, x, ldx, gamma, beta, y, ldy, rows, C, act, lens, t_per_batch, yh, yl, ldh);
    else if (C <= 1024) hipLaunchKernelGGL((layernorm_kernel<4>), grid, dim3(256), 0, s, x, ldx, gamma, beta, y, ldy, rows, C, act, lens, t_per_batch, yh, yl, ldh);
    else hipLaunchKernelGGL((layernorm_kernel<16>), grid, dim3(256), 0, s, x, ldx, gamma, beta, y, ldy, rows, C, act, lens, t_per_batch, yh, yl, ldh);
    SC_LAUNCH_CHECK();
}

void launch_layernorm(const float* x, int64_t ldx, const float* gamma, const float* beta, float* y,
                      int64_t ldy, int rows, int C, int act, const int* lens, int t_per_batch,
                      hipStream_t s) {
    SC_CHECK(C % 4 == 0 && ldx % 4 == 0 && ldy % 4 == 0, "layernorm: C=%d ldx=%lld ldy=%lld must be multiples of 4", C,
             (long long)ldx, (long long)ldy);
    SC_CHECK(C <= 4096, "layernorm: C=%d > 4096 unsupported", C);
    if (rows <= 0) return;
    dim3 grid(cdiv(rows, 4));
    if (C <= 256) {
        hipLaunchKernelGGL((layernorm_kernel<1>), grid, dim3(256), 0, s, x, ldx, gamma, beta, y, ldy, rows, C, act, lens, t_per_batch, (__half*)nullptr, (__half*)nullptr, (int64_t)0);
    } else if (C <= 1024) {
        hipLaunchKernelGGL((layernorm_kernel<4>), grid, dim3(256), 0, s, x, ldx, gamma, beta, y, ldy, rows, C, act, lens, t_per_batch, (__half*)nullptr, (__half*)nullptr, (int64_t)0);
    } else {
        hipLaunchKernelGGL((layernorm_kernel<16>), grid, dim3(256), 0, s, x, ldx, gamma, beta, y, ldy, rows, C, act, lens, t_per_batch, (__half*)nullptr, (__half*)nullptr, (int64_t)0);
    }
    SC_LAUNCH_CHECK();
}

__global__ __launch_bounds__(256) void glu_kernel(const float* __restrict__ x, int64_t ldx,
                                                  float* __restrict__ y, int64_t ldy, int rows, int C) {
    const int cv = C >> 2;
    const int64_t total = (int64_t)rows * cv;
    for (int64_t i = (int64_t)blockIdx.x * blockDim.x + threadIdx.x; i < total;
         i += (int64_t)gridDim.x * blockDim.x) {
        const int r = (int)(i / cv);
        const int c = (int)(i - (int64_t)r * cv);
        const float4 a = *reinterpret_cast<const float4*>(x + (int64_t)r * ldx + c * 4);
        const float4 g = *reinterpret_cast<const float4*>(x + (int64_t)r * ldx + C + c * 4);
        float4 o;
        o.x = a.x / (1.f + expf(-g.x));
        o.y = a.y / (1.f + expf(-g.y));
        o.z = a.z / (1.f + expf(-g.z));
        o.w = a.w / (1.f + expf(-g.w));
        *reinterpret_cast<float4*>(y + (int64_t)r * ldy + c * 4) = o;
    }
}

void launch_glu(const float* x, int64_t ldx, float* y, int64_t ldy, int rows, int C, hipStream_t s) {
    SC_CHECK(C % 4 == 0 && ldx % 4 == 0 && ldy % 4 == 0, "glu: alignment");
    if (rows <= 0) return;
    const int64_t total = (int64_t)rows * (C / 4);
    const int blocks = (int)std::min<int64_t>(cdiv64(total, 256), 4096);
    hipLaunchKernelGGL(glu_kernel, dim3(blocks), dim3(256), 0, s, x, ldx, y, ldy, rows, C);
    SC_LAUNCH_CHECK();
}

template <int K, int TT>
__global__ __launch_bounds__(256) void glu_dwconv_kernel(const float* __restrict__ x, int64_t ldx,
                                                         const float* __restrict__ w,
                                                         float* __restrict__ y, int64_t ldy, int T,
                                                         int C, const int* __restrict__ lens, int left,
                                                         const float* __restrict__ bn_scale,
                                                         const float* __restrict__ bn_shift) {
    const int c = blockIdx.x * 256 + threadIdx.x;
    const int t0 = blockIdx.y * TT;
    const int n = blockIdx.z;
    if (c >= C) return;
    const int len = lens ? min(lens[n], T) : T;
    float wr[K];
#pragma unroll
    for (int j = 0; j < K; ++j) wr[j] = w[c * K + j];
    float g[TT + K - 1];
#pragma unroll
    for (int i = 0; i < TT + K - 1; ++i) {
// ... 2 lines not shown
        if (t >= 0 && t < len) {
            const float* xr = x + ((int64_t)n * T + t) * ldx;
            const float a = xr[c];
            const float b = xr[C + c];
            v = a / (1.f + expf(-b));
        }
        g[i] = v;
    }
#pragma unroll
    for (int tt = 0; tt < TT; ++tt) {
        const int t = t0 + tt;
        if (t < T) {
            float acc = 0.f;
#pragma unroll
            for (int j = 0; j < K; ++j) acc = fmaf(wr[j], g[tt + j], acc);
            if (bn_scale) {
                acc = fmaf(acc, bn_scale[c], bn_shift[c]);
                acc = acc / (1.f + expf(-acc));
            }
            y[((int64_t)n * T + t) * ldy + c] = acc;
        }
    }
}

__global__ __launch_bounds__(256) void glu_dwconv_generic_kernel(const float* __restrict__ x, int64_t ldx,
                                                                 const float* __restrict__ w,
                                                                 float* __restrict__ y, int64_t ldy,
                                                                 int T, int C, int K,
                                                                 const int* __restrict__ lens, int left,
                                                                 const float* __restrict__ bn_scale,
                                                                 const float* __restrict__ bn_shift) {
    const int c = blockIdx.x * 256 + threadIdx.x;
    const int t = blockIdx.y;
    const int n = blockIdx.z;
    if (c >= C) return;
    const int len = lens ? min(lens[n], T) : T;
    float acc = 0.f;
    for (int j = 0; j < K; ++j) {
        const int ts = t - left + j;
        if (ts >= 0 && ts < len) {
            const float* xr = x + ((int64_t)n * T + ts) * ldx;
            acc = fmaf(w[c * K + j], xr[c] / (1.f + expf(-xr[C + c])), acc);
        }
    }
    if (bn_scale) {
        acc = fmaf(acc, bn_scale[c], bn_shift[c]);
        acc = acc / (1.f + expf(-acc));
    }
    y[((int64_t)n * T + t) * ldy + c] = acc;
}

__global__ void bn_fold_kernel(const float* __restrict__ g, const float* __restrict__ b, const float* __restrict__ mean,
                               const float* __restrict__ var, float eps, int C, float* __restrict__ scale, float* __restrict__ shift) {
    const int c = blockIdx.x * blockDim.x + threadIdx.x;
    if (c >= C) return;
    const float sc = g[c] / sqrtf(var[c] + eps);
    scale[c] = sc;
    shift[c] = b[c] - mean[c] * sc;
}

void launch_bn_fold(const float* g, const float* b, const float* mean, const float* var, float eps, int C, float* scale, float* shift,
                    hipStream_t s) {
    hipLaunchKernelGGL(bn_fold_kernel, dim3(cdiv(C, 256)), dim3(256), 0, s, g, b, mean, var, eps, C, scale, shift);
    SC_LAUNCH_CHECK();
}

__global__ void relpos_table_kernel(int S, int M, float* __restrict__ out) {
    const int idx = blockIdx.x * blockDim.x + threadIdx.x;
    const int half = M / 2;
    if (idx >= (2 * S - 1) * half) return;
    const int t = idx / half, i = idx - t * half;
    const float pos = (float)((S - 1) - t);
    const float div = expf((float)(2 * i) * -(logf(10000.0f) / (float)M));
    const float a = pos * div;
    out[(int64_t)t * M + 2 * i] = sinf(a);
    out[(int64_t)t * M + 2 * i + 1] = cosf(a);
}

void launch_relpos_table(int S, int M, float* out, hipStream_t s) {
    hipLaunchKernelGGL(relpos_table_kernel, dim3(cdiv((2 * S - 1) * (M / 2), 256)), dim3(256), 0, s, S, M, out);
    SC_LAUNCH_CHECK();
}

template <int K, int TT>
__global__ __launch_bounds__(1024) void glu_dwconv_ln_kernel(const float* __restrict__ x, int64_t ldx, const float* __restrict__ w,
                                                             const float* __restrict__ gamma, const float* __restrict__ beta, int act,
                                                             __half* __restrict__ yh, __half* __restrict__ yl, int64_t ldh, int T, int C,
                                                             const int* __restrict__ lens, int range) {
    __shared__ float tile[2][TT][1024];
    typedef _Float16 h4_t __attribute__((ext_vector_type(4)));
    typedef float f4_t __attribute__((ext_vector_type(4)));
    const int c = threadIdx.x;
    const int lane = c & 63, wv = c >> 6, waves = C >> 6;
    const int n = blockIdx.y;
    const int t_begin = blockIdx.x * range, t_end = min(T, t_begin + range);
    if (t_begin >= t_end) return;
    const int len = lens ? min(lens[n], T) : T;
    const float* xn = x + (int64_t)n * T * ldx;
    float wr[K];
#pragma unroll
    for (int j = 0; j < K; ++j) wr[j] = w[c * K + j];
    float g[TT + K - 1];
#pragma unroll
    for (int i = 0; i < K - 1; ++i) {
        const int t = t_begin - (K - 1) + i;
        float v = 0.f;
        if (t >= 0 && t < len) {
            const float a = xn[(int64_t)t * ldx + c];
            const float b = xn[(int64_t)t * ldx + C + c];
            v = a / (1.f + expf(-b));
        }
        g[i] = v;
    }
    float ra[TT], rb[TT];
#pragma unroll
    for (int i = 0; i < TT; ++i) {
        const int t = t_begin + i;
        const bool ok = t < t_end && t < len;
        ra[i] = ok ? xn[(int64_t)t * ldx + c] : 0.f;
        rb[i] = ok ? xn[(int64_t)t * ldx + C + c] : 0.f;
    }
    const int nv = C >> 2;
    int buf = 0;
    for (int tc = t_begin; tc < t_end; tc += TT) {
#pragma unroll
        for (int i = 0; i < TT; ++i) {
            const int t = tc + i;
            g[K - 1 + i] = (t < t_end && t < len) ? ra[i] / (1.f + expf(-rb[i])) : 0.f;
        }
#pragma unroll
        for (int i = 0; i < TT; ++i) {
            const int t = tc + TT + i;
            const bool ok = t < t_end && t < len;
            ra[i] = ok ? xn[(int64_t)t * ldx + c] : 0.f;
            rb[i] = ok ? xn[(int64_t)t * ldx + C + c] : 0.f;
        }
#pragma unroll
        for (int tt = 0; tt < TT; ++tt) {
            float acc = 0.f;
#pragma unroll
            for (int j = 0; j < K; ++j) acc = fmaf(wr[j], g[tt + j], acc);
            tile[buf][tt][c] = acc;
        }
        __syncthreads();
        for (int r = wv; r < TT && tc + r < t_end; r += waves) {
            const float4* xr = reinterpret_cast<const float4*>(&tile[buf][r][0]);
            const int64_t row = (int64_t)n * T + tc + r;
            h4_t* yhr = reinterpret_cast<h4_t*>(yh + row * ldh);
            h4_t* ylr = reinterpret_cast<h4_t*>(yl + row * ldh);
            float s = 0.f;
#pragma unroll
            for (int i = 0; i < 4; ++i) {
                const int idx = lane + 64 * i;
                const float4 vv = idx < nv ? xr[idx] : make_float4(0.f, 0.f, 0.f, 0.f);
                s += (vv.x + vv.y) + (vv.z + vv.w);
            }
            const float mean = wave_sum(s) / (float)C;
            float q = 0.f;
#pragma unroll
            for (int i = 0; i < 4; ++i) {
                const int idx = lane + 64 * i;
                if (idx < nv) {
                    const float4 vv = xr[idx];
                    const float a = vv.x - mean, b = vv.y - mean, cc = vv.z - mean, d = vv.w - mean;
                    q += (a * a + b * b) + (cc * cc + d * d);
                }
            }
            const float var = wave_sum(q) / (float)C;
            const float rstd = 1.0f / sqrtf(var + 1e-5f);
            const float4* g4 = reinterpret_cast<const float4*>(gamma);
            const float4* b4 = reinterpret_cast<const float4*>(beta);
#pragma unroll
            for (int i = 0; i < 4; ++i) {
                const int idx = lane + 64 * i;
                if (idx < nv) {
                    const float4 gg = g4[idx], bb = b4[idx], vv = xr[idx];
                    float4 o;
                    o.x = act_f((vv.x - mean) * rstd * gg.x + bb.x, act);
                    o.y = act_f((vv.y - mean) * rstd * gg.y + bb.y, act);
                    o.z = act_f((vv.z - mean) * rstd * gg.z + bb.z, act);
                    o.w = act_f((vv.w - mean) * rstd * gg.w + bb.w, act);
                    const f4_t of = {o.x, o.y, o.z, o.w};
                    const h4_t hi = __builtin_convertvector(of, h4_t);
                    const f4_t back = __builtin_convertvector(hi, f4_t);
                    yhr[idx] = hi;
                    ylr[idx] = __builtin_convertvector(of - back, h4_t);
                }
            }
        }
#pragma unroll
        for (int i = 0; i < K - 1; ++i) g[i] = g[i + TT];
        buf ^= 1;
    }
}

bool glu_dwconv_ln_supported(int C, int ksize) { return ksize == 31 && C % 64 == 0 && C >= 64 && C <= 1024; }

void launch_glu_dwconv_ln(const float* x, int64_t ldx, const float* w, const float* gamma, const float* beta, int act, __half* yh,
                          __half* yl, int64_t ldh, int nb, int T, int C, int ksize, const int* lens, hipStream_t s) {
    SC_CHECK(glu_dwconv_ln_supported(C, ksize) && ldh % 4 == 0, "glu_dwconv_ln: C=%d k=%d ldh=%lld unsupported", C, ksize, (long long)ldh);
    if (nb <= 0 || T <= 0) return;
    constexpr int TT = 8;
    int ranges = std::max(1, std::min(cdiv(256, nb), cdiv(T, 32)));
    const int range = cdiv(cdiv(T, ranges), TT) * TT;
    ranges = cdiv(T, range);
    const double rows = (double)nb * T;
    prof::Scope scope("glu_dwconv_ln", 2.0 * rows * C * ksize, rows * C * (8.0 + 4.0), s);
    hipLaunchKernelGGL((glu_dwconv_ln_kernel<31, TT>), dim3(ranges, nb), dim3(C), 0, s, x, ldx, w, gamma, beta, act, yh, yl, ldh, T, C, lens,
                       range);
    SC_LAUNCH_CHECK();
}

void launch_glu_dwconv(const float* x, int64_t ldx, const float* w, float* y, int64_t ldy, int nb, int T,
                       int C, int ksize, const int* lens, hipStream_t s, int left, const float* bn_scale, const float* bn_shift) {
    if (nb <= 0 || T <= 0) return;
    if (left < 0) left = ksize - 1;
    if (ksize == 31) {
        constexpr int TT = 16;
        dim3 grid(cdiv(C, 256), cdiv(T, TT), nb);
        hipLaunchKernelGGL((glu_dwconv_kernel<31, TT>), grid, dim3(256), 0, s, x, ldx, w, y, ldy, T, C, lens, left, bn_scale, bn_shift);
    } else {
        dim3 grid(cdiv(C, 256), T, nb);
        hipLaunchKernelGGL(glu_dwconv_generic_kernel, grid, dim3(256), 0, s, x, ldx, w, y, ldy, T, C, ksize, lens, left, bn_scale, bn_shift);
    }
    SC_LAUNCH_CHECK();
}

}
```

### seamless_communication_amd/csrc/kernels.h

```cpp
#pragma once
#include <atomic>

#include "common.h"
#include "prof.h"

namespace sc {

enum Act { ACT_NONE = 0, ACT_RELU = 1, ACT_SILU = 2, ACT_TANH = 3, ACT_GELU = 4 };
enum InAct { IN_NONE = 0, IN_LRELU_01 = 1, IN_LRELU_001 = 2 };

struct GemmArgs {
    const float* A = nullptr;
    int64_t lda = 0;
    const __half* W = nullptr;
    int64_t ldw = 0;
    int64_t w_phase_stride = 0;
    const float* bias = nullptr;
    const float* res = nullptr;
    int64_t ldr = 0;
    float* C = nullptr;
    int64_t ldc = 0;
    int M = 0;
    int N = 0;
    int K = 0;
    int rows_per_batch = 0;
    int t_in = 0;
    int t_out = 0;
    int taps = 1, cin = 0, dil = 0, stride = 1, pad = 0;
    int out_mul = 1, out_off = 0, out_off_phase_step = 0;
    const int* in_lens = nullptr;
    int in_act = IN_NONE;
    int act = ACT_NONE;
    float alpha = 1.0f;
    int phases = 1;
    int split = 1;
    double algo_flops = 0;
    const int* item_off = nullptr;
    int n_items = 0, item_mul = 1, item_extra = 0, item_out_mul = 1;
};

#if defined(__HIPCC__)
template <typename F>
__device__ __forceinline__ int item_search(int n, int key, F first) {
    int lo = 0, hi = n - 1;
    while (lo < hi) {
        const int mid = (lo + hi + 1) >> 1;
        if (first(mid) <= key) lo = mid;
        else hi = mid - 1;
    }
    return lo;
}

struct GemmItemCursor {
    int n = 0, start = 0, next = 0x7fffffff;
    __device__ __forceinline__ static int first(const GemmArgs& p, int i) { return p.item_off[i] * p.item_mul + i * p.item_extra; }
    __device__ __forceinline__ void init(const GemmArgs& p, int m) {
        n = item_search(p.n_items, m, [&](int i) { return first(p, i); });
        start = first(p, n);
        next = first(p, n + 1);
    }
    __device__ __forceinline__ void seek(const GemmArgs& p, int m) {
        while (m >= next) {
            ++n;
            start = next;
            next = first(p, n + 1);
        }
    }
    __device__ __forceinline__ int q(int m) const { return m - start; }
    __device__ __forceinline__ int in_row0(const GemmArgs& p) const { return start - n * p.item_extra; }
    __device__ __forceinline__ int t_in(const GemmArgs& p) const { return next - start - p.item_extra; }
    __device__ __forceinline__ int t_out(const GemmArgs& p) const { return t_in(p) * p.item_out_mul; }
    __device__ __forceinline__ int64_t out_row0(const GemmArgs& p) const { return (int64_t)in_row0(p) * p.item_out_mul; }
};
#endif

void launch_gemm(const GemmArgs& a, hipStream_t s);
extern std::atomic<int> g_force_general_gemm;
bool gemm_fast_eligible(const GemmArgs& a);
void launch_gemm_fast(const GemmArgs& a, hipStream_t s);

struct GemmPsArgs {
    const __half* Ah = nullptr;
    const __half* Al = nullptr;
    int64_t lda = 0;
    const __half* W = nullptr;
    int64_t ldw = 0;
    const float* bias = nullptr;
    const float* res = nullptr;
    int64_t ldr = 0;
    float* C = nullptr;
    int64_t ldc = 0;
    __half* Ch = nullptr;
    __half* Cl = nullptr;
    int64_t ldcs = 0;
    int M = 0, N = 0, K = 0;
    int act = ACT_NONE;
    float alpha = 1.0f;
    int split = 1;
    float plane_neg_slope = 1.0f;
    int conv_taps = 0, conv_cin = 0, conv_dil = 1, conv_pad = 0, rows_per_item = 0;
    const unsigned char* row_valid = nullptr;
    const int2* row_pos = nullptr;
    float2* amax = nullptr;
    int amax_ld = 0;
};
void launch_gemm_presplit(const GemmPsArgs& a, hipStream_t s);
int gemm_presplit_amax_chunks(int M, int N);
void launch_amax_finish(const float2* part, int ld, int rows, int* out_idx, hipStream_t s);

struct ResPairArgs {
    const float* x = nullptr;
    float* out = nullptr;
    const __half* w1 = nullptr;
    int64_t ldw1 = 0;
    const float* b1 = nullptr;
    const __half* w2 = nullptr;
    int64_t ldw2 = 0;
    const float* b2 = nullptr;
    int nb = 0, T = 0, C = 0, k = 0, dil = 1;
    float slope = 0.1f;
    const float* avg_a = nullptr;
    const float* avg_b = nullptr;
    int single = 0;
    const int* item_off = nullptr;
    const int* tile_first = nullptr;
    int item_mul = 1, total_tiles = 0;
};
bool resblock_pair_supported(int C, int k, int dil);
int resblock_pair_tile_rows(int k);
void launch_resblock_pair(const ResPairArgs& a, hipStream_t s);

struct MrfArgs {
    const float* x = nullptr;
    float* out = nullptr;
    int nb = 0, T = 0, C = 0;
    float slope = 0.1f;
    int halo = 0;
    int k[3] = {0, 0, 0};
    int dil[9] = {1, 1, 1, 1, 1, 1, 1, 1, 1};
    const __half* w1[9] = {};
    const __half* w2[9] = {};
    int64_t ldw1[9] = {};
    int64_t ldw2[9] = {};
    const float* b1[9] = {};
    const float* b2[9] = {};
    int single = 0;
    const int* item_off = nullptr;
    const int* tile_first = nullptr;
    int item_mul = 1, total_tiles = 0;
};
bool mrf_fused_supported(int C, const int* k, const int* dil);
int mrf_tile_rows(const int* k, const int* dil);
void launch_mrf_fused(const MrfArgs& a, hipStream_t s);

void launch_gemv(const float* x, int64_t ldx, const __half* W, int64_t ldw, const float* bias,
                 const float* res, int64_t ldr, float* out, int64_t ldo, int M, int N, int K,
                 int act, float alpha, hipStream_t s);

struct SkinnyArgs {
    const float* A = nullptr;
    int64_t lda = 0;
    const __half* W = nullptr;
    int64_t ldw = 0;
    const float* bias = nullptr;
    const float* res = nullptr;
    int64_t ldr = 0;
    float* C = nullptr;
    int64_t ldc = 0;
    float* partial = nullptr;
    int M = 0, N = 0, K = 0;
    int act = ACT_NONE;
    float alpha = 1.0f;
    int splits = 1;
    int kc = 0;
    float4* am_part = nullptr;
    int am_tiles_cap = 0;
    int am_tiles = 0;
    float* am_eos_logit = nullptr;
    const int* am_pos = nullptr;
    int am_min_step_for_eos = 0, am_force_eos_step = -1;
    int am_pad_idx = -1, am_eos_idx = -1, am_unk_idx = -1;
    float am_unk_penalty = 0.f;
};
int skinny_argmax_tiles(int M, int N);
void launch_argmax_finalize(const float4* part, int tiles, int nb, const float* eos_logit, const int* d_pos,
                            int force_eos_step, int pad_idx, int eos_idx, int* next_tok, int* hist, int hist_ld,
                            int* finished, int* out_len, float* score, hipStream_t s);
void launch_skinny(const SkinnyArgs& a, hipStream_t s);
int skinny_splits(int M, int N, int K, int want_split);
// ... 99 lines not shown
    __half* Oh = nullptr;
    __half* Ol = nullptr;
    int ORB = 32;
    int act = ACT_NONE;
    const int* d_rows = nullptr;
    int KS = 0, NT_total = 0;
    uint32_t w_bytes = 0, a_bytes = 0;
    int xcd_swizzle = 0, touch = 0;
};
enum Gemv3Shape { G3_T1 = 0, G3_T2K8 = 1, G3_T2K4 = 2 };
bool gemv3_supported(int M, int N, int K, int in_mode);
int gemv3_splits(int K, int shape);
void launch_gemv3(const Gemv3Args& a, hipStream_t s);
struct Reduce3Args {
    const float* partial = nullptr;
    int S = 0;
    const float* bias = nullptr;
    float* xg = nullptr;
    int XRB = 32;
    const float* gamma = nullptr;
    const float* beta = nullptr;
    __half* Hh = nullptr;
    __half* Hl = nullptr;
    int RB = 32;
    float* hrow = nullptr;
    int64_t hrow_bs = 0;
    int hrow_rows = 0;
    const int* d_pos = nullptr;
    float* hfix = nullptr;
    int rows = 0, C = 0;
    const int* d_rows = nullptr;
    const int2* slot_rp = nullptr;
};
void launch_reduce3(const Reduce3Args& a, hipStream_t s);
void launch_embed3(const int* tok, const __half* embed, float scale, const float* pos_table, const int* d_pos, float* xg, int XRB,
                   int rows, int C, hipStream_t s, const int2* slot_rp = nullptr, const int* d_rows = nullptr);
void launch_ln3(const float* xg, int XRB, const float* gamma, const float* beta, __half* Hh, __half* Hl, int RB, int rows, int C,
                hipStream_t s);
void launch_rows_to_kgm(const float* x, int64_t ldx, int rows, int C, int XRB, float* xg, hipStream_t s);
void launch_kgm_to_rows(const float* xg, int XRB, float* out, int64_t ldo, int rows, int C, hipStream_t s);
struct Vocab3Args {
    const __half* Wp = nullptr;
    const __half* Ah = nullptr;
    const __half* Al = nullptr;
    int RB = 32;
    int M = 0, N = 0, K = 0;
    const float* bias = nullptr;
    float* logits = nullptr;
    int64_t ldl = 0;
    float4* am_part = nullptr;
    int am_tiles_cap = 0;
    float* am_eos_logit = nullptr;
    const int* am_pos = nullptr;
    int am_min_step_for_eos = 0, am_force_eos_step = -1;
    int am_pad_idx = -1, am_eos_idx = -1, am_unk_idx = -1;
    float am_unk_penalty = 0.f;
    const int* d_rows = nullptr;
    const int2* slot_rp = nullptr;
    const int* limit_row = nullptr;
    int KS = 0, NT_total = 0, tpg = 0, halves = 1;
    uint32_t w_bytes = 0;
};
bool vocab3_supported(int M, int N, int K);
int vocab3_groups(int M);
void launch_vocab3(const Vocab3Args& a, hipStream_t s);

void launch_layernorm(const float* x, int64_t ldx, const float* gamma, const float* beta, float* y,
                      int64_t ldy, int rows, int C, int act, const int* lens, int t_per_batch,
                      hipStream_t s);

void launch_layernorm_split(const float* x, int64_t ldx, const float* gamma, const float* beta, __half* yh, __half* yl,
                            int64_t ldh, int rows, int C, int act, const int* lens, int t_per_batch, hipStream_t s);
void launch_layernorm2_split(const float* x, int64_t ldx, const float* ga, const float* ba, float* y, int64_t ldy, const float* gb2,
                             const float* bb2, __half* yh, __half* yl, int64_t ldh, int rows, int C, hipStream_t s);
void launch_layernorm_both(const float* x, int64_t ldx, const float* gamma, const float* beta, float* y, int64_t ldy, __half* yh,
                           __half* yl, int64_t ldh, int rows, int C, int act, const int* lens, int t_per_batch, hipStream_t s);
void launch_lrelu_split_f32(const float* x, float neg_slope, __half* hi, __half* lo, int64_t n, hipStream_t s);
void launch_split_f32(const float* x, __half* hi, __half* lo, int64_t n, hipStream_t s);

void launch_glu(const float* x, int64_t ldx, float* y, int64_t ldy, int rows, int C, hipStream_t s);

bool glu_dwconv_ln_supported(int C, int ksize);
void launch_glu_dwconv_ln(const float* x, int64_t ldx, const float* w, const float* gamma, const float* beta, int act, __half* yh,
                          __half* yl, int64_t ldh, int nb, int T, int C, int ksize, const int* lens, hipStream_t s);
void launch_glu_dwconv(const float* x, int64_t ldx, const float* w, float* y, int64_t ldy, int nb, int T,
                       int C, int ksize, const int* lens, hipStream_t s, int left = -1, const float* bn_scale = nullptr,
                       const float* bn_shift = nullptr);
void launch_bn_fold(const float* g, const float* b, const float* mean, const float* var, float eps, int C, float* scale, float* shift,
                    hipStream_t s);
void launch_relpos_table(int S, int M, float* out, hipStream_t s);

struct AttnArgs {
    const float* q = nullptr;
    const float* k = nullptr;
    const float* v = nullptr;
    float* out = nullptr;
    int64_t ldq = 0, ldk = 0, ldv = 0, ldo = 0;
    int nb = 0, heads = 0, Sq = 0, Skv = 0;
    const int* kv_lens = nullptr;
    int causal = 0;
    const float* rel_k = nullptr;
    int rel_left = 0, rel_right = 0;
    const float* rp_table = nullptr;
    int64_t rp_ld = 0;
    const float* q_bias_u = nullptr;
    const float* q_bias_v = nullptr;
    const int* row_off = nullptr;
    double pairs = 0;
    __half* out_hi = nullptr;
    __half* out_lo = nullptr;
    int64_t ldoh = 0;
    int head_dim = 64;
};
void launch_attention(const AttnArgs& a, hipStream_t s);
void launch_attention80(const AttnArgs& a, hipStream_t s);

void launch_decode_attention(const float* q, int64_t ldq, const float* k_new, const float* v_new,
                             int64_t ldkv, float* kcache, float* vcache, int64_t cache_ld, int64_t cache_bs,
                             int cap, float* out, int64_t ldo, int nb, int heads, const int* d_pos,
                             const int* kv_lens, int use_lens, hipStream_t s, int in_splits = 1,
                             int64_t in_split_stride = 0, const float* bias_q = nullptr,
                             const float* bias_k = nullptr, const float* bias_v = nullptr);

constexpr int BANNED_MAX_SEQS = 4096, BANNED_MAX_LEN = 64, BANNED_MAX_TOKENS = 65536;
struct BannedList {
    const int* tokens = nullptr;
    const int* offsets = nullptr;
    int n = 0;
    int max_len = 0;
};
void validate_banned_host(const int32_t* tokens, const int32_t* offsets, int n_banned, int V, int* out_max_len);
void launch_beam_candidates(float* logits, int64_t ld, int n_utt, int beams, int V, const float* cum, int first_step,
                            int no_eos, int force_eos, int pad_idx, int eos_idx, int unk_idx, float unk_penalty, int K,
                            float* cand_val, int* cand_idx, const int* seqs, int seq_ld, int S, int G, hipStream_t s,
                            const int* d_slots = nullptr, const BannedList* banned = nullptr);
bool beam_chunked(int V, int beams, int K);
size_t beam_ws_floats(int rows, int K);
size_t beam_ws_ints(int rows, int K);
void launch_beam_candidates_chunked(float* logits, int64_t ld, int n_utt, int beams, int V, const float* cum, int first_step, int no_eos,
                                    int force_eos, int pad_idx, int eos_idx, int unk_idx, float unk_penalty, int K, float* cand_val,
                                    int* cand_idx, const int* seqs, int seq_ld, int S, int G, float* ws_f, int* ws_i, hipStream_t s,
                                    const int* d_rows = nullptr, const int* d_slots = nullptr, const BannedList* banned = nullptr);
struct BeamSelectArgs {
    const float* cand_val = nullptr;
    const int* cand_idx = nullptr;
    const int* seqs_cur = nullptr;
    int* seqs_new = nullptr;
    float* fin_score = nullptr;
    int* fin_len = nullptr;
    int* fin_seq = nullptr;
    int* fin_count = nullptr;
    int* done = nullptr;
    int* remaining = nullptr;
    int* tok = nullptr;
    int* src_row = nullptr;
    float* cum = nullptr;
    int* anc = nullptr;
    int anc_ld = 0;
    const int* slot_utt = nullptr;
    const int* d_slots = nullptr;
    int beams = 0, K = 0, V = 0, max_len = 0, step = 0;
    int eos_idx = 0, pad_idx = 0, normalize = 1;
    float len_penalty = 1.f;
};
void launch_beam_select(const BeamSelectArgs& a, int n_utt, hipStream_t s);
struct BeamCompactArgs {
    const int* done = nullptr;
// ... 191 lines not shown
```

### seamless_communication_amd/csrc/model.h

```cpp
#pragma once
#include <algorithm>
#include <map>
#include <functional>
#include <memory>
#include <string>
#include <unordered_map>
#include <vector>

#include "../../include/seamless_hip.h"
#include "kernels.h"

namespace sc {

class DevicePool {
   public:
    ~DevicePool();
    void* get(size_t bytes);
    void put(void* p);
    void release_all();
    void trim();
    void set_stream(hipStream_t s) { stream_ = s; }
    void set_oom_hook(std::function<void()> f) { oom_hook_ = std::move(f); }

   private:
    std::function<void()> oom_hook_;
    void* debug_filled(void* p, size_t bytes);
    hipStream_t stream_ = nullptr;
    std::multimap<size_t, void*> free_;
    std::unordered_map<void*, size_t> size_;
    size_t cached_bytes_ = 0;
};

template <typename T>
class Buf {
   public:
    Buf() = default;
    Buf(DevicePool* pool, size_t n) : pool_(pool), n_(n) { p_ = n ? static_cast<T*>(pool->get(n * sizeof(T))) : nullptr; }
    Buf(const Buf&) = delete;
    Buf& operator=(const Buf&) = delete;
    Buf(Buf&& o) noexcept : pool_(o.pool_), p_(o.p_), n_(o.n_) { o.p_ = nullptr; }
    Buf& operator=(Buf&& o) noexcept {
        if (this != &o) {
            reset();
            pool_ = o.pool_;
            p_ = o.p_;
            n_ = o.n_;
            o.p_ = nullptr;
        }
        return *this;
    }
    ~Buf() { reset(); }
    void reset() {
        if (p_) pool_->put(p_);
        p_ = nullptr;
    }
    T* get() const { return p_; }
    operator T*() const { return p_; }
    size_t size() const { return n_; }

   private:
    DevicePool* pool_ = nullptr;
    T* p_ = nullptr;
    size_t n_ = 0;
};

struct Linear {
    const __half* w = nullptr;
    const __half* wp = nullptr;
    int64_t ldw = 0;
    const float* b = nullptr;
    int out = 0, in = 0, kpad = 0;
};
struct LNorm {
    const float* g = nullptr;
    const float* b = nullptr;
    int dim = 0;
};
struct Conv {
    const __half* w = nullptr;
    const float* b = nullptr;
    int cout = 0, cin = 0, k = 0, kpad = 0;
};
struct ConvT {
    const __half* w = nullptr;
    const float* b = nullptr;
    int cin = 0, cout = 0, k = 0, stride = 0, pad = 0, taps = 0, kpad = 0;
};

struct ConformerLayer {
    LNorm ffn1_ln, attn_ln, conv_ln, conv_inner_ln, ffn2_ln, final_ln;
    Linear ffn1_in, ffn1_out, ffn2_in, ffn2_out, qkv, attn_out, pw1, pw2;
    const float* rel_k = nullptr;
    const float* dw = nullptr;
    Linear r_proj;
    const float* u_bias = nullptr;
    const float* v_bias = nullptr;
    const float* bn_scale = nullptr;
    const float* bn_shift = nullptr;
};
struct AdaptorLayer {
    LNorm res_ln, attn_ln, ffn_ln;
    Conv res_conv, attn_conv;
    Linear qkv, attn_out, ffn_in, ffn_out;
};
struct DecoderLayer {
    LNorm self_ln, cross_ln, ffn_ln;
    Linear qkv, self_out, cross_q, cross_kv, cross_out, ffn_in, ffn_out;
};
struct PChooseLayer {
    std::vector<Linear> q, k;
    const float* energy_bias = nullptr;
};
struct DecStack {
    const __half* embed = nullptr;
    const __half* embed_p = nullptr;
    const float* pos = nullptr;
    const std::vector<DecoderLayer>* layers = nullptr;
    const LNorm* final_ln = nullptr;
    int ffn_dim = 0;
    const std::vector<PChooseLayer>* pchoose = nullptr;
    int vocab = 0, pad_idx = 0, unk_idx = 1, eos_idx = 3, max_seq_len = 0;
};
struct EncoderLayer {
    LNorm attn_ln, ffn_ln;
    Linear qkv, attn_out, ffn_in, ffn_out;
};
struct FFTLayer {
    Linear qkv, attn_out;
    LNorm attn_ln, conv_ln;
    Conv conv1, conv2;
};
struct ResBlock {
    std::vector<Conv> convs1, convs2;
    std::vector<int> dil;
};

struct ModelData {
    sc_config cfg{};
    int device = 0;

    struct Raw {
        void* p;
        int dtype;
        std::vector<int64_t> shape;
        int64_t numel;
    };
    std::unordered_map<std::string, Raw> raw;

    float* fbank_consts = nullptr;
    LNorm fe_ln;
    Linear fe_proj;
    std::vector<ConformerLayer> enc;
    LNorm enc_inner_ln, enc_final_ln;
    Linear enc_proj1, enc_proj2;
    AdaptorLayer adaptor;
    const __half* text_embed = nullptr;
    const __half* text_embed_p = nullptr;
    const float* text_pos = nullptr;
    std::vector<DecoderLayer> dec;
    LNorm dec_final_ln;
    const __half* mma_embed = nullptr;
    const __half* mma_embed_p = nullptr;
    std::vector<DecoderLayer> mma_dec;
    std::vector<PChooseLayer> mma_pc;
    const __half* const* mma_qe_w = nullptr;
    const float* const* mma_qe_b = nullptr;
    const float* const* mma_ebias = nullptr;
    const __half* const* mma_ke_w = nullptr;
    const float* const* mma_ke_b = nullptr;
    int mma_qe_ldw = 0;
    LNorm mma_final_ln;
    std::vector<EncoderLayer> text_enc;
    LNorm text_enc_ln;
    std::vector<EncoderLayer> t2u_enc;
// ... 184 lines not shown
```

### seamless_communication_amd/csrc/model_encoder.hip

```cpp
#include <cstdlib>

#include <cmath>
#include "model.h"

namespace sc {

static void upload_i32(Model& m, int* d, const int32_t* h, int n) {
    SC_HIP(hipMemcpyAsync(d, h, (size_t)n * 4, hipMemcpyHostToDevice, m.stream));
}

static void fbank_geometry(int sample_rate, int& frame_len, int& frame_shift, int& nfft) {
    frame_len = (int)((float)sample_rate * 0.001f * 25.0f);
    frame_shift = (int)((float)sample_rate * 0.001f * 10.0f);
    nfft = 1;
    while (nfft < frame_len) nfft *= 2;
}

int fbank_num_frames(int64_t num_samples, int sample_rate) {
    int fl, fs, nf;
    fbank_geometry(sample_rate, fl, fs, nf);
    return num_samples < fl ? 0 : (int)(1 + (num_samples - fl) / fs);
}

static const Model::FbankRate& fbank_rate_consts(Model& m, int sample_rate) {
// ... 55 lines not shown
    }
    if (standardize) launch_standardize(d_out, n, t_rows, d_fr, m.cfg.num_fbank_channels, m.stream);
    SC_HIP(hipStreamSynchronize(m.stream));
}

static int adaptor_len(const sc_config& c, int len) {
    const int pad = c.adaptor_kernel_size / 2;
    const double v = (double)(len + 2 * pad - c.adaptor_kernel_size) / (double)c.adaptor_stride + 1.0;
    return (int)std::floor(v);
}

int encoder_out_len(const Model& m, int t_frames) {
    const sc_config& c = m.cfg;
    const int S = t_frames / c.fbank_stride;
    const int pad = c.adaptor_kernel_size / 2;
    return (S + 2 * pad - c.adaptor_kernel_size) / c.adaptor_stride + 1;
}

static void attention_self(Model& m, const float* qkv, int Mdim, float* out, int nb, int S, const int* d_lens,
                           const float* rel_k) {
    AttnArgs a;
    a.q = qkv;
    a.k = qkv + Mdim;
    a.v = qkv + 2 * Mdim;
    a.out = out;
    a.ldq = a.ldk = a.ldv = 3 * Mdim;
    a.ldo = Mdim;
    a.nb = nb;
    a.heads = m.cfg.num_heads;
    a.Sq = S;
    a.Skv = S;
    a.kv_lens = d_lens;
    a.rel_k = rel_k;
    a.rel_left = rel_k ? m.cfg.shaw_max_left : 0;
    a.rel_right = rel_k ? m.cfg.shaw_max_right : 0;
    launch_attention(a, m.stream);
}

void run_encode_speech(Model& m, const float* d_fbank, int n, int t_frames, const int32_t* h_lens, float* d_out,
                       int32_t* h_out_lens) {
    const sc_config& c = m.cfg;
    const int M = c.model_dim;
    SC_CHECK(n > 0 && t_frames > 0, "sc_encode_speech: empty batch");
    prof::set_tag("enc");
    SC_CHECK(t_frames % c.fbank_stride == 0, "sc_encode_speech: t_frames=%d must be a multiple of fbank_stride=%d (Collater pad_to_multiple)",
             t_frames, c.fbank_stride);
    const int S = t_frames / c.fbank_stride;
    const int rows = n * S;
    const int feat = c.num_fbank_channels * c.fbank_stride;
    std::vector<int32_t> lens(n), alens(n);
    for (int i = 0; i < n; ++i) {
        SC_CHECK(h_lens[i] >= 0 && h_lens[i] <= t_frames, "sc_encode_speech: frame_lens[%d]=%d out of range", i, h_lens[i]);
        lens[i] = h_lens[i] / c.fbank_stride;
        alens[i] = adaptor_len(c, lens[i]);
        if (h_out_lens) h_out_lens[i] = alens[i];
    }
    Buf<int> d_lens(m.pp(), n), d_alens(m.pp(), n);
    upload_i32(m, d_lens, lens.data(), n);
    upload_i32(m, d_alens, alens.data(), n);

    const int F = std::max(std::max(c.enc_ffn_dim, c.adaptor_proj_dim), std::max(3 * M, c.adaptor_ffn_dim));
    Buf<float> x(m.pp(), (size_t)rows * M), h(m.pp(), (size_t)rows * std::max(M, feat)), wide(m.pp(), (size_t)rows * F),
        att(m.pp(), (size_t)rows * M);

    launch_layernorm(d_fbank, feat, m.fe_ln.g, m.fe_ln.b, h, feat, rows, feat, ACT_NONE, nullptr, 1, m.stream);
    linear(m, h, feat, m.fe_proj, nullptr, 0, x, M, rows, ACT_NONE, 1.f);

    static const bool presplit = knob::value("SC_PRESPLIT", 1) != 0;
    const bool v1 = c.enc_variant == 1;
    const bool ps_ok = !v1 && presplit && M % 32 == 0 && c.enc_ffn_dim % 32 == 0 && (int64_t)rows * std::max(M, c.enc_ffn_dim) * 2 < (1ll << 31);
    Buf<float> rp_tab(m.pp(), v1 ? (size_t)(2 * S - 1) * M : 0), rp_proj(m.pp(), v1 ? (size_t)(2 * S - 1) * M : 0);
    if (v1) launch_relpos_table(S, M, rp_tab, m.stream);
    Buf<__half> hs(m.pp(), ps_ok ? (size_t)2 * rows * M : 0), ws(m.pp(), ps_ok ? (size_t)2 * rows * c.enc_ffn_dim : 0),
        as(m.pp(), ps_ok ? (size_t)2 * rows * M : 0);
    __half* hs_hi = hs.get();
    __half* hs_lo = ps_ok ? hs.get() + (size_t)rows * M : nullptr;
    __half* ws_hi = ws.get();
    __half* ws_lo = ps_ok ? ws.get() + (size_t)rows * c.enc_ffn_dim : nullptr;
    __half* as_hi = as.get();
    __half* as_lo = ps_ok ? as.get() + (size_t)rows * M : nullptr;
    auto ln_split = [&](const float* src, const LNorm& L, int act) {
        launch_layernorm_split(src, L.dim, L.g, L.b, hs_hi, hs_lo, L.dim, rows, L.dim, act, nullptr, 1, m.stream);
    };
    auto ps = [&](const __half* ah, const __half* al, const Linear& L, int act, float alpha, const float* res, float* C,
                  __half* Ch, __half* Cl) {
        GemmPsArgs a;
        a.Ah = ah;
        a.Al = al;
        a.lda = L.in;
        a.W = L.w;
        a.ldw = L.ldw;
        a.bias = L.b;
        a.res = res;
        a.ldr = L.out;
        a.C = C;
        a.ldc = L.out;
        a.Ch = Ch;
        a.Cl = Cl;
        a.ldcs = L.out;
        a.M = rows;
        a.N = L.out;
        a.K = L.in;
        a.act = act;
        a.alpha = alpha;
        static const bool single = knob::value("SC_SPLIT_MODE", 0) == 1;
        a.split = single ? 0 : 1;
        launch_gemm_presplit(a, m.stream);
    };

    static const bool fuse = knob::value("SC_ENC_FUSE", 1) != 0;
    const bool fuse_conv = fuse && glu_dwconv_ln_supported(M, c.depthwise_conv_kernel_size);
    const bool fuse_ln = fuse && M <= 1024;
    bool ffn1_planes_ready = false;
    for (int li = 0; li < c.enc_layers; ++li) {
        const ConformerLayer& l = m.enc[li];
        if (ps_ok) {
            if (!ffn1_planes_ready) ln_split(x, l.ffn1_ln, ACT_NONE);
            ps(hs_hi, hs_lo, l.ffn1_in, ACT_SILU, 1.f, nullptr, nullptr, ws_hi, ws_lo);
            ps(ws_hi, ws_lo, l.ffn1_out, ACT_NONE, 0.5f, x, x, nullptr, nullptr);
            ln_split(x, l.attn_ln, ACT_NONE);
            ps(hs_hi, hs_lo, l.qkv, ACT_NONE, 1.f, nullptr, wide, nullptr, nullptr);
            {
                AttnArgs a;
                a.q = wide;
                a.k = wide.get() + M;
                a.v = wide.get() + 2 * M;
                a.out_hi = as_hi;
                a.out_lo = as_lo;
                a.ldoh = M;
                a.ldq = a.ldk = a.ldv = 3 * M;
                a.ldo = M;
                a.nb = n;
                a.heads = c.num_heads;
                a.Sq = S;
                a.Skv = S;
                a.kv_lens = d_lens;
                a.rel_k = l.rel_k;
                a.rel_left = c.shaw_max_left;
                a.rel_right = c.shaw_max_right;
                launch_attention(a, m.stream);
            }
            ps(as_hi, as_lo, l.attn_out, ACT_NONE, 1.f, x, x, nullptr, nullptr);
            ln_split(x, l.conv_ln, ACT_NONE);
            ps(hs_hi, hs_lo, l.pw1, ACT_NONE, 1.f, nullptr, wide, nullptr, nullptr);
            if (fuse_conv) {
                launch_glu_dwconv_ln(wide, 2 * M, l.dw, l.conv_inner_ln.g, l.conv_inner_ln.b, ACT_SILU, hs_hi, hs_lo, M, n, S, M,
                                     c.depthwise_conv_kernel_size, d_lens, m.stream);
            } else {
                launch_glu_dwconv(wide, 2 * M, l.dw, att, M, n, S, M, c.depthwise_conv_kernel_size, d_lens, m.stream);
                ln_split(att, l.conv_inner_ln, ACT_SILU);
            }
            ps(hs_hi, hs_lo, l.pw2, ACT_NONE, 1.f, x, x, nullptr, nullptr);
            ln_split(x, l.ffn2_ln, ACT_NONE);
            ps(hs_hi, hs_lo, l.ffn2_in, ACT_SILU, 1.f, nullptr, nullptr, ws_hi, ws_lo);
            ps(ws_hi, ws_lo, l.ffn2_out, ACT_NONE, 0.5f, x, x, nullptr, nullptr);
            if (fuse_ln && li + 1 < c.enc_layers) {
                const LNorm& nx = m.enc[li + 1].ffn1_ln;
                launch_layernorm2_split(x, M, l.final_ln.g, l.final_ln.b, x, M, nx.g, nx.b, hs_hi, hs_lo, M, rows, M, m.stream);
                ffn1_planes_ready = true;
            } else {
                layernorm(m, x, l.final_ln, x, rows);
                ffn1_planes_ready = false;
            }
            continue;
        }
        layernorm(m, x, l.ffn1_ln, h, rows);
        linear(m, h, M, l.ffn1_in, nullptr, 0, wide, c.enc_ffn_dim, rows, ACT_SILU, 1.f);
        linear(m, wide, c.enc_ffn_dim, l.ffn1_out, x, M, x, M, rows, ACT_NONE, 0.5f);
        layernorm(m, x, l.attn_ln, h, rows);
        linear(m, h, M, l.qkv, nullptr, 0, wide, 3 * M, rows, ACT_NONE, 1.f);
        if (v1) {
            linear(m, rp_tab, M, l.r_proj, nullptr, 0, rp_proj, M, 2 * S - 1, ACT_NONE, 1.f);
            AttnArgs a;
            a.q = wide;
            a.k = wide.get() + M;
            a.v = wide.get() + 2 * M;
            a.out = att;
            a.ldq = a.ldk = a.ldv = 3 * M;
            a.ldo = M;
            a.nb = n;
            a.heads = c.num_heads;
            a.Sq = S;
            a.Skv = S;
            a.kv_lens = d_lens;
            a.rp_table = rp_proj;
            a.rp_ld = M;
            a.q_bias_u = l.u_bias;
            a.q_bias_v = l.v_bias;
            launch_attention(a, m.stream);
        } else {
            attention_self(m, wide, M, att, n, S, d_lens, l.rel_k);
        }
        linear(m, att, M, l.attn_out, x, M, x, M, rows, ACT_NONE, 1.f);
        layernorm(m, x, l.conv_ln, h, rows);
        linear(m, h, M, l.pw1, nullptr, 0, wide, 2 * M, rows, ACT_NONE, 1.f);
        if (v1) {
            launch_glu_dwconv(wide, 2 * M, l.dw, h, M, n, S, M, c.depthwise_conv_kernel_size, d_lens, m.stream,
                              c.depthwise_conv_kernel_size / 2, l.bn_scale, l.bn_shift);
        } else {
            launch_glu_dwconv(wide, 2 * M, l.dw, att, M, n, S, M, c.depthwise_conv_kernel_size, d_lens, m.stream);
            layernorm(m, att, l.conv_inner_ln, h, rows, ACT_SILU);
        }
        linear(m, h, M, l.pw2, x, M, x, M, rows, ACT_NONE, 1.f);
        layernorm(m, x, l.ffn2_ln, h, rows);
        linear(m, h, M, l.ffn2_in, nullptr, 0, wide, c.enc_ffn_dim, rows, ACT_SILU, 1.f);
        linear(m, wide, c.enc_ffn_dim, l.ffn2_out, x, M, x, M, rows, ACT_NONE, 0.5f);
        layernorm(m, x, l.final_ln, x, rows);
    }
    layernorm(m, x, m.enc_inner_ln, x, rows);
    linear(m, x, M, m.enc_proj1, nullptr, 0, wide, c.adaptor_proj_dim, rows, ACT_RELU, 1.f);
    linear(m, wide, c.adaptor_proj_dim, m.enc_proj2, x, M, x, M, rows, ACT_NONE, 0.5f);

    const AdaptorLayer& a = m.adaptor;
    const int Sa = encoder_out_len(m, t_frames);
    const int arows = n * Sa;
    const int k = c.adaptor_kernel_size, st = c.adaptor_stride, pad = k / 2;
    Buf<float> res(m.pp(), (size_t)arows * M), y(m.pp(), (size_t)arows * M), conv(m.pp(), (size_t)arows * 2 * M),
        aw(m.pp(), (size_t)arows * std::max(3 * M, c.adaptor_ffn_dim)), ah(m.pp(), (size_t)arows * M);
    layernorm(m, x, a.res_ln, h, rows);
    conv1d(m, h, a.res_conv, nullptr, conv, n, S, st, pad, 1, nullptr, IN_NONE, ACT_NONE);
    launch_glu(conv, 2 * M, res, M, arows, M, m.stream);
    layernorm(m, x, a.attn_ln, h, rows);
    conv1d(m, h, a.attn_conv, nullptr, conv, n, S, st, pad, 1, nullptr, IN_NONE, ACT_NONE);
    launch_glu(conv, 2 * M, y, M, arows, M, m.stream);
    linear(m, y, M, a.qkv, nullptr, 0, aw, 3 * M, arows, ACT_NONE, 1.f);
    attention_self(m, aw, M, ah, n, Sa, d_alens, nullptr);
    linear(m, ah, M, a.attn_out, res, M, y, M, arows, ACT_NONE, 1.f);
    layernorm(m, y, a.ffn_ln, ah, arows);
    linear(m, ah, M, a.ffn_in, nullptr, 0, aw, c.adaptor_ffn_dim, arows, ACT_RELU, 1.f);
    linear(m, aw, c.adaptor_ffn_dim, a.ffn_out, y, M, y, M, arows, ACT_NONE, 1.f);
    launch_layernorm(y, M, m.enc_final_ln.g, m.enc_final_ln.b, d_out, M, arows, M, ACT_NONE, nullptr, 1, m.stream);
    SC_HIP(hipStreamSynchronize(m.stream));
}
// ... 3 lines not shown
```

### seamless_communication_amd/csrc/model_load.hip

```cpp
#include <cmath>
#include <cstring>

#include <cstdlib>

#include "model.h"

namespace sc {

DevicePool::~DevicePool() { release_all(); }

static int debug_fill_byte() {
    static const int v = [] {
        (void)knob::is_set("SC_DEBUG_FILL");
        const char* e = getenv("SC_DEBUG_FILL");
        return e && *e ? (int)strtol(e, nullptr, 0) & 0xff : -1;
    }();
    return v;
}

void* DevicePool::debug_filled(void* p, size_t bytes) {
    const int v = debug_fill_byte();
    if (v >= 0 && p && stream_) {
        hipStreamCaptureStatus st = hipStreamCaptureStatusNone;
        if (hipStreamIsCapturing(stream_, &st) == hipSuccess && st == hipStreamCaptureStatusNone)
// ... 265 lines not shown
    for (int i = 0; i < 400; ++i) c[i] = (float)std::pow(0.5 - 0.5 * std::cos(a * (double)i), 0.85);
    auto mel_scale = [](float f) { return 1127.0f * logf(1.0f + f / 700.0f); };
    const float nyquist = 8000.0f, fft_bin_width = 16000.0f / 512.0f;
    const float mel_low = mel_scale(20.0f), mel_high = mel_scale(nyquist);
    const float delta = (mel_high - mel_low) / (80 + 1);
    float* melT = c.data() + 400;
    for (int b = 0; b < 80; ++b) {
        const float left = mel_low + b * delta, center = mel_low + (b + 1) * delta, right = mel_low + (b + 2) * delta;
        for (int i = 0; i < 256; ++i) {
            const float mel = mel_scale(fft_bin_width * i);
            if (mel > left && mel < right) {
                float w;
                if (mel <= center) w = (mel - left) / (center - left);
                else w = (right - mel) / (right - center);
                melT[i * 80 + b] = w;
            }
        }
    }
    float* tw = c.data() + 400 + 256 * 80;
    for (int k = 0; k < 256; ++k) {
        tw[k] = (float)std::cos(-2.0 * M_PI * k / 512.0);
        tw[256 + k] = (float)std::sin(-2.0 * M_PI * k / 512.0);
    }
    void* d = nullptr;
    SC_HIP(hipMalloc(&d, c.size() * 4));
    m.owned.push_back(d);
    SC_HIP(hipMemcpy(d, c.data(), c.size() * 4, hipMemcpyHostToDevice));
    m.fbank_consts = static_cast<float*>(d);
}

}

void load_model(Model& m, const sc_tensor_desc* t, size_t n) {
    const sc_config& c = m.cfg;
    SC_CHECK(c.model_dim == c.num_heads * 64, "sc_load: head_dim must be 64 (model_dim=%d, heads=%d)", c.model_dim,
             c.num_heads);
    SC_CHECK(c.model_dim % 32 == 0, "sc_load: model_dim must be a multiple of 32");
    std::unordered_map<const void*, void*> seen;
    for (size_t i = 0; i < n; ++i) {
        const sc_tensor_desc& d = t[i];
        SC_CHECK(d.name && d.data && d.ndim >= 0 && d.ndim <= 4, "sc_load: bad tensor descriptor #%zu", i);
        SC_CHECK(d.dtype == SC_F16 || d.dtype == SC_F32, "sc_load: tensor '%s' has unsupported dtype %d", d.name, d.dtype);
        Model::Raw r;
        r.dtype = d.dtype;
        r.numel = 1;
        for (int k = 0; k < d.ndim; ++k) {
            r.shape.push_back(d.shape[k]);
            r.numel *= d.shape[k];
        }
        const size_t bytes = (size_t)r.numel * (d.dtype == SC_F16 ? 2 : 4);
        auto it = seen.find(d.data);
        if (it != seen.end()) {
            r.p = it->second;
        } else {
            void* p = nullptr;
            SC_HIP(hipMalloc(&p, std::max<size_t>(bytes, 256)));
            m.owned.push_back(p);
            SC_HIP(hipMemcpy(p, d.data, bytes, d.on_device ? hipMemcpyDeviceToDevice : hipMemcpyHostToDevice));
            r.p = p;
            seen[d.data] = p;
        }
        m.raw[d.name] = std::move(r);
    }
    Loader L(m);
    const int M = c.model_dim;
    build_fbank_consts(m);

    const int feat = c.num_fbank_channels * c.fbank_stride;
    m.fe_ln = L.ln("speech_encoder_frontend.post_extract_layer_norm", feat);
    m.fe_proj = L.lin("speech_encoder_frontend.model_dim_proj", M, feat);
    const int npos = c.shaw_max_left + 1 + c.shaw_max_right;
    m.enc.resize(c.enc_layers);
    for (int i = 0; i < c.enc_layers; ++i) {
        const std::string p = "speech_encoder.inner.layers." + std::to_string(i);
        ConformerLayer& l = m.enc[i];
        l.ffn1_ln = L.ln(p + ".ffn1_layer_norm", M);
        l.ffn1_in = L.lin(p + ".ffn1.inner_proj", c.enc_ffn_dim, M);
        l.ffn1_out = L.lin(p + ".ffn1.output_proj", M, c.enc_ffn_dim);
        l.attn_ln = L.ln(p + ".self_attn_layer_norm", M);
        l.qkv = L.fuse({p + ".self_attn.q_proj", p + ".self_attn.k_proj", p + ".self_attn.v_proj"}, M, M);
        l.attn_out = L.lin(p + ".self_attn.output_proj", M, M);
        l.conv_ln = L.ln(p + ".conv_layer_norm", M);
        l.pw1 = L.lin_pw(p + ".conv.pointwise_conv1", 2 * M, M);
        l.dw = L.f32(p + ".conv.depthwise_conv.weight", {M, 1, c.depthwise_conv_kernel_size});
        if (c.enc_variant == 1) {
            l.r_proj = L.lin(p + ".self_attn.sdpa.r_proj", M, M, false);
            l.u_bias = L.f32(p + ".self_attn.sdpa.u_bias", {c.num_heads, 64});
            l.v_bias = L.f32(p + ".self_attn.sdpa.v_bias", {c.num_heads, 64});
            const float* g = L.f32(p + ".conv.batch_norm.weight", {M});
            const float* b = L.f32(p + ".conv.batch_norm.bias", {M});
            const float* mu = L.f32(p + ".conv.batch_norm.running_mean", {M});
            const float* var = L.f32(p + ".conv.batch_norm.running_var", {M});
            float* fold = static_cast<float*>(L.dalloc((size_t)2 * M * 4));
            launch_bn_fold(g, b, mu, var, 1e-5f, M, fold, fold + M, m.stream);
            l.bn_scale = fold;
            l.bn_shift = fold + M;
        } else {
            l.rel_k = L.f32(p + ".self_attn.sdpa.rel_k_embed.weight", {npos, 64});
            l.conv_inner_ln = L.ln(p + ".conv.layer_norm", M);
        }
        l.pw2 = L.lin_pw(p + ".conv.pointwise_conv2", M, M);
        l.ffn2_ln = L.ln(p + ".ffn2_layer_norm", M);
        l.ffn2_in = L.lin(p + ".ffn2.inner_proj", c.enc_ffn_dim, M);
        l.ffn2_out = L.lin(p + ".ffn2.output_proj", M, c.enc_ffn_dim);
        l.final_ln = L.ln(p + ".layer_norm", M);
    }
    m.enc_inner_ln = L.ln("speech_encoder.inner_layer_norm", M);
    m.enc_proj1 = L.lin("speech_encoder.proj1", c.adaptor_proj_dim, M);
    m.enc_proj2 = L.lin("speech_encoder.proj2", M, c.adaptor_proj_dim);
    {
        const std::string p = "speech_encoder.adaptor_layers.0";
        AdaptorLayer& a = m.adaptor;
        a.res_ln = L.ln(p + ".residual_layer_norm", M);
        a.res_conv = L.conv(p + ".residual_conv", 2 * M, M, c.adaptor_kernel_size);
        a.attn_ln = L.ln(p + ".self_attn_layer_norm", M);
        a.attn_conv = L.conv(p + ".self_attn_conv", 2 * M, M, c.adaptor_kernel_size);
        a.qkv = L.fuse({p + ".self_attn.q_proj", p + ".self_attn.k_proj", p + ".self_attn.v_proj"}, M, M);
        a.attn_out = L.lin(p + ".self_attn.output_proj", M, M);
        a.ffn_ln = L.ln(p + ".ffn_layer_norm", M);
        a.ffn_in = L.lin(p + ".ffn.inner_proj", c.adaptor_ffn_dim, M);
        a.ffn_out = L.lin(p + ".ffn.output_proj", M, c.adaptor_ffn_dim);
    }
    m.enc_final_ln = L.ln("speech_encoder.layer_norm", M);

    m.text_embed = L.f16("text_decoder_frontend.embed.weight", {c.text_vocab_size, M});
    m.text_pos = L.f32("text_decoder_frontend.pos_encoder.freqs", {c.text_max_seq_len, M});
    m.dec.resize(c.dec_layers);
    for (int i = 0; i < c.dec_layers; ++i) {
        const std::string p = "text_decoder.layers." + std::to_string(i);
        DecoderLayer& l = m.dec[i];
        l.self_ln = L.ln(p + ".self_attn_layer_norm", M);
        l.qkv = L.fuse({p + ".self_attn.q_proj", p + ".self_attn.k_proj", p + ".self_attn.v_proj"}, M, M);
        l.self_out = L.lin(p + ".self_attn.output_proj", M, M);
        l.cross_ln = L.ln(p + ".encoder_decoder_attn_layer_norm", M);
        l.cross_q = L.lin(p + ".encoder_decoder_attn.q_proj", M, M);
        l.cross_kv = L.fuse({p + ".encoder_decoder_attn.k_proj", p + ".encoder_decoder_attn.v_proj"}, M, M);
        l.cross_out = L.lin(p + ".encoder_decoder_attn.output_proj", M, M);
        l.ffn_ln = L.ln(p + ".ffn_layer_norm", M);
        l.ffn_in = L.lin(p + ".ffn.inner_proj", c.dec_ffn_dim, M);
        l.ffn_out = L.lin(p + ".ffn.output_proj", M, c.dec_ffn_dim);
        L.pack_decoder_layer(l);
    }
    m.text_embed_p = L.packed(m.text_embed, M, c.text_vocab_size, M);
    m.dec_final_ln = L.ln("text_decoder.layer_norm", M);

    SC_CHECK(c.mma_layers >= 0 && c.mma_energy_layers >= 0, "sc_load: mma_layers=%d mma_energy_layers=%d", c.mma_layers,
             c.mma_energy_layers);
    if (c.mma_layers > 0) {
        SC_CHECK(c.mma_energy_layers >= 1 && c.mma_pre_decision_ratio >= 1 && c.mma_temperature > 0.f,
                 "sc_load: monotonic decoder needs energy layers / pre_decision_ratio / temperature");
        const std::string root = "monotonic_decoder.";
        m.mma_embed = L.f16(root + "text_decoder_frontend.embed.weight", {c.text_vocab_size, M});
        m.mma_dec.resize(c.mma_layers);
        m.mma_pc.resize(c.mma_layers);
        for (int i = 0; i < c.mma_layers; ++i) {
            const std::string p = root + "text_decoder.layers." + std::to_string(i);
            DecoderLayer& l = m.mma_dec[i];
            l.self_ln = L.ln(p + ".self_attn_layer_norm", M);
            l.qkv = L.fuse({p + ".self_attn.q_proj", p + ".self_attn.k_proj", p + ".self_attn.v_proj"}, M, M);
            l.self_out = L.lin(p + ".self_attn.output_proj", M, M);
            l.cross_ln = L.ln(p + ".encoder_decoder_attn_layer_norm", M);
            l.cross_q = L.lin(p + ".encoder_decoder_attn.q_proj", M, M);
            l.cross_kv = L.fuse({p + ".encoder_decoder_attn.k_proj", p + ".encoder_decoder_attn.v_proj"}, M, M);
            l.cross_out = L.lin(p + ".encoder_decoder_attn.output_proj", M, M);
            l.ffn_ln = L.ln(p + ".ffn_layer_norm", M);
            l.ffn_in = L.lin(p + ".ffn.inner_proj", c.mma_ffn_dim, M);
// ... 341 lines not shown
```

Before: 334.8.

## Fuse Conformer conv-module GLU into the first pointwise GEMM epilogue

At load time the first pointwise-conv weight is reordered so each 64-row block interleaves 32 value rows with their 32 gate rows. The presplit GEMM gets a GLU epilogue that applies value*sigmoid(gate) inside the tile and writes only C columns. The following depthwise-conv+LN kernel then reads the gated half-width tensor instead of the 2C-wide output. This removes half of the intermediate write and read traffic, at the cost of a second reordered weight copy in memory and forcing a tile of at least 128.

```diff
diff --git a/include/seamless_hip_internal.h b/include/seamless_hip_internal.h
--- a/include/seamless_hip_internal.h
+++ b/include/seamless_hip_internal.h
@@ -80,6 +80,9 @@
                      const int32_t* d_lens);
 int sc_op_glu_dwconv_ln(const float* d_x, const float* d_w, const float* d_gamma, const float* d_beta, int32_t act, void* d_yh_f16,
                         void* d_yl_f16, int32_t nb, int32_t T, int32_t C, int32_t k, const int32_t* d_lens, int32_t fused);
+int sc_op_pw1_glu(const float* d_x, const void* d_w_f16, const float* d_bias, float* d_y, const float* d_dw, const float* d_gamma,
+                  const float* d_beta, int32_t act, void* d_yh_f16, void* d_yl_f16, int32_t nb, int32_t T, int32_t C, int32_t K,
+                  const int32_t* d_lens, int32_t mode);
 int sc_op_layernorm2(const float* d_x, const float* d_ga, const float* d_ba, const float* d_gb, const float* d_bb, float* d_y,
                      void* d_yh_f16, void* d_yl_f16, int32_t rows, int32_t C, int32_t fused);
 int sc_op_argmax(const float* d_logits, int32_t rows, int32_t V, int32_t* d_idx, float* d_lprob);
diff --git a/seamless_communication_amd/_lib.py b/seamless_communication_amd/_lib.py
--- a/seamless_communication_amd/_lib.py
+++ b/seamless_communication_amd/_lib.py
@@ -199,6 +199,7 @@
     "sc_op_dstep_argmax": (C.c_int, [_P, _P, _i, _i, _i, _i, _i, _i, _i, _i, _i, C.c_float, _i, _P, _P]),
     "sc_op_resblock_pair_ps": (C.c_int, [_P, _P, _P, _P, _P, _P, _i, _i, _i, _i, _i]),
     "sc_op_glu_dwconv_ln": (C.c_int, [_P, _P, _P, _P, _i, _P, _P, _i, _i, _i, _i, _P, _i]),
+    "sc_op_pw1_glu": (C.c_int, [_P, _P, _P, _P, _P, _P, _P, _i, _P, _P, _i, _i, _i, _i, _P, _i]),
     "sc_op_layernorm2": (C.c_int, [_P, _P, _P, _P, _P, _P, _P, _P, _i, _i, _i]),
     "sc_op_dstep3_gemv": (C.c_int, [_i, _P, _P, _P, _P, _P, _P, _P, _P, _i, _i, _i, _i, _i, _i]),
     "sc_op_dstep3_argmax": (C.c_int, [_P, _P, _i, _i, _i, _i, _i, _i, _i, _i, _i, C.c_float, _P, _P]),
diff --git a/seamless_communication_amd/csrc/api.hip b/seamless_communication_amd/csrc/api.hip
--- a/seamless_communication_amd/csrc/api.hip
+++ b/seamless_communication_amd/csrc/api.hip
@@ -1413,6 +1413,52 @@
     SC_API_END
 }
 
+int sc_op_pw1_glu(const float* d_x, const void* d_w_f16, const float* d_bias, float* d_y, const float* d_dw, const float* d_gamma,
+                  const float* d_beta, int32_t act, void* d_yh_f16, void* d_yl_f16, int32_t nb, int32_t T, int32_t C, int32_t K,
+                  const int32_t* d_lens, int32_t mode) {
+    SC_API_BEGIN
+    SC_CHECK(d_x && d_w_f16 && (d_y || d_dw) && (!d_dw || (d_gamma && d_beta && d_yh_f16 && d_yl_f16)), "sc_op_pw1_glu: null argument");
+    SC_CHECK(mode == 0 || mode == 1 || mode == 128 || mode == 256, "sc_op_pw1_glu: mode %d", mode);
+    const int rows = nb * T;
+    OpScratch scratch;
+    __half* hi = scratch.get<__half>((size_t)rows * K);
+    __half* lo = scratch.get<__half>((size_t)rows * K);
+    launch_split_f32(d_x, hi, lo, (int64_t)rows * K, g_op_stream);
+    GemmPsArgs a;
+    a.Ah = hi;
+    a.Al = lo;
+    a.lda = K;
+    a.W = static_cast<const __half*>(d_w_f16);
+    a.ldw = K;
+    a.bias = d_bias;
+    a.M = rows;
+    a.N = 2 * C;
+    a.K = K;
+    __half* yh = static_cast<__half*>(d_yh_f16);
+    __half* yl = static_cast<__half*>(d_yl_f16);
+    if (mode == 0) {
+        float* wide = scratch.get<float>((size_t)rows * 2 * C);
+        a.C = wide;
+        a.ldc = 2 * C;
+        launch_gemm_presplit(a, g_op_stream);
+        if (d_y) launch_glu(wide, 2 * C, d_y, C, rows, C, g_op_stream);
+        if (d_dw) launch_glu_dwconv_ln(wide, 2 * C, d_dw, d_gamma, d_beta, act, yh, yl, C, nb, T, C, 31, d_lens, g_op_stream);
+    } else {
+        __half* wg = scratch.get<__half>((size_t)2 * C * K);
+        launch_glu_row_order(a.W, K, wg, C, K, g_op_stream);
+        float* gated = d_y ? d_y : scratch.get<float>((size_t)rows * C);
+        a.W = wg;
+        a.C = gated;
+        a.ldc = C;
+        a.glu = 1;
+        a.glu_tile = mode == 1 ? 0 : mode;
+        launch_gemm_presplit(a, g_op_stream);
+        if (d_dw) launch_glu_dwconv_ln(gated, C, d_dw, d_gamma, d_beta, act, yh, yl, C, nb, T, C, 31, d_lens, g_op_stream, true);
+    }
+    SC_HIP(hipStreamSynchronize(g_op_stream));
+    SC_API_END
+}
+
 int sc_op_layernorm2(const float* d_x, const float* d_ga, const float* d_ba, const float* d_gb, const float* d_bb, float* d_y,
                      void* d_yh_f16, void* d_yl_f16, int32_t rows, int32_t C, int32_t fused) {
     SC_API_BEGIN
diff --git a/seamless_communication_amd/csrc/common.cpp b/seamless_communication_amd/csrc/common.cpp
--- a/seamless_communication_amd/csrc/common.cpp
+++ b/seamless_communication_amd/csrc/common.cpp
@@ -47,6 +47,7 @@
     {"SC_VOC_PACKED", 0, "0: ragged vocoder batches in length buckets on side chains instead of the packed pass"},
     {"SC_VOC_PACK_ROWS", 0, "vocoder: unit rows per packed group"},
     {"SC_ENGINE_RG_SMALL", 0, "decode engine: rows per row group, N = 1024 products"},
+    {"SC_ENC_GLU_EP", 2, "Conformer conv module: GLU in the first pointwise product's epilogue (0 off, 1 where the product's tile has it, 2 always)"},
     {"SC_BEAM_COMPACT", 2, "0: beam search keeps finished utterances' slots"},
     {"SC_GREEDY_COMPACT", 2, "0: greedy generation keeps finished rows in their slots"}, {"SC_GREEDY_POLL", 2, "steps between looks at the finished flags"},
 };
diff --git a/seamless_communication_amd/csrc/k_gemm_ps.hip b/seamless_communication_amd/csrc/k_gemm_ps.hip
--- a/seamless_communication_amd/csrc/k_gemm_ps.hip
+++ b/seamless_communication_amd/csrc/k_gemm_ps.hip
@@ -35,7 +35,7 @@
 
 __device__ __forceinline__ int swz(int row, int s) { return row * 64 + ((s ^ ((row >> 2) & 3)) << 4); }
 
-template <int WM, int WN, int EP_LD, int ACT>
+template <int WM, int WN, int EP_LD, int ACT, bool RAW = false>
 __device__ __forceinline__ void ps_epilogue(const GemmPsArgs& p, const float* ep, int m0w, int n0w, int lane) {
     typedef float f4_t __attribute__((ext_vector_type(4)));
     typedef _Float16 h4_t __attribute__((ext_vector_type(4)));
@@ -51,7 +51,7 @@
     const int col = n0w + c0;
     const bool vec_ok = (col + 3 < p.N) && ((p.ldc | p.ldr | p.ldcs) % 4 == 0) && (n0w % 4 == 0);
     f4_t b4 = {0.f, 0.f, 0.f, 0.f};
-    if (p.bias) {
+    if (!RAW && p.bias) {
 #pragma unroll
         for (int e = 0; e < 4; ++e) b4[e] = (col + e < p.N) ? p.bias[col + e] : 0.f;
     }
@@ -61,12 +61,12 @@
         const int64_t m = m0w + row;
         const f4_t a = *reinterpret_cast<const f4_t*>(ep + row * EP_LD + c0);
         if (m >= p.M || col >= p.N) continue;
-        const bool dead = p.row_valid && p.row_valid[m] == 0;
+        const bool dead = !RAW && p.row_valid && p.row_valid[m] == 0;
         f4_t v;
 #pragma unroll
-        for (int e = 0; e < 4; ++e) v[e] = dead ? 0.f : ps_act<ACT>(a[e] + b4[e]) * p.alpha;
+        for (int e = 0; e < 4; ++e) v[e] = RAW ? a[e] : dead ? 0.f : ps_act<ACT>(a[e] + b4[e]) * p.alpha;
         if (vec_ok) {
-            if (p.res && !dead) v += *reinterpret_cast<const f4_t*>(p.res + m * p.ldr + col);
+            if (!RAW && p.res && !dead) v += *reinterpret_cast<const f4_t*>(p.res + m * p.ldr + col);
             if (p.C) *reinterpret_cast<f4_t*>(p.C + m * p.ldc + col) = v;
             if (p.Ch) {
                 if (p.plane_neg_slope != 1.0f) {
@@ -84,7 +84,7 @@
             for (int e = 0; e < 4; ++e) {
                 if (col + e >= p.N) continue;
                 float x = v[e];
-                if (p.res && !dead) x += p.res[m * p.ldr + col + e];
+                if (!RAW && p.res && !dead) x += p.res[m * p.ldr + col + e];
                 if (p.C) p.C[m * p.ldc + col + e] = x;
                 if (p.Ch) {
                     if (p.plane_neg_slope != 1.0f) x = fmaxf(x, 0.f) + p.plane_neg_slope * fminf(x, 0.f);
@@ -97,9 +97,9 @@
     }
 }
 
-template <int BM, int BN, int WGM, int WGN, bool SPLIT, bool CONV, bool AMAX>
-__global__ __launch_bounds__(WGM* WGN * 64) void gemm_ps_kernel(GemmPsArgs p, int tiles_n, int tiles_total, int tiles_per_xcd,
-                                                                 uint32_t a_bytes, uint32_t w_bytes) {
+template <int BM, int BN, int WGM, int WGN, bool SPLIT, bool CONV, bool AMAX, bool GLU>
+__device__ __forceinline__ void gemm_ps_body(const GemmPsArgs& p, int tiles_n, int tiles_total, int tiles_per_xcd, uint32_t a_bytes,
+                                             uint32_t w_bytes) {
     constexpr int NWAVE = WGM * WGN;
     constexpr bool ALTERNATE = SPLIT && NWAVE == 8;
     constexpr bool MID_BARRIER = SPLIT && !ALTERNATE;
@@ -455,14 +455,40 @@
     int am_idx = 0x7fffffff;
     auto pass = [&](auto hc) {
         constexpr int h = decltype(hc)::value;
-#pragma unroll
-        for (int i = 0; i < TM; ++i)
-#pragma unroll
-            for (int j = 0; j < EPN / 32; ++j)
-#pragma unroll
-                for (int r = 0; r < 16; ++r)
-                    ep[(i * 32 + (r & 3) + 8 * (r >> 2) + 4 * (lane >> 5)) * EP_LD + j * 32 + (lane & 31)] = acc[i][h * (EPN / 32) + j][r];
         const int n0w = n0 + wn * WN + h * EPN;
+        if constexpr (GLU) {
+            static_assert(EPN % 64 == 0 && !AMAX, "a pass holds whole (value, gate) pairs of 32-column blocks");
+            GemmPsArgs q = p;
+            q.N = p.N >> 1;
+            const int oc0 = n0w >> 1;
+#pragma unroll
+            for (int jp = 0; jp < EPN / 64; ++jp) {
+                const int oc = oc0 + jp * 32 + (lane & 31);
+                float ba = 0.f, bb = 0.f;
+                if (p.bias && oc < q.N) {
+                    ba = p.bias[oc];
+                    bb = p.bias[q.N + oc];
+                }
+#pragma unroll
+                for (int i = 0; i < TM; ++i)
+#pragma unroll
+                    for (int r = 0; r < 16; ++r) {
+                        const float a = acc[i][h * (EPN / 32) + 2 * jp][r] + ba;
+                        const float b = acc[i][h * (EPN / 32) + 2 * jp + 1][r] + bb;
+                        ep[(i * 32 + (r & 3) + 8 * (r >> 2) + 4 * (lane >> 5)) * EP_LD + jp * 32 + (lane & 31)] = a / (1.f + expf(-b));
+                    }
+            }
+            ps_epilogue<WM, EPN / 2, EP_LD, ACT_NONE, true>(q, ep, m0w, oc0, lane);
+            return;
+        } else {
+#pragma unroll
+            for (int i = 0; i < TM; ++i)
+#pragma unroll
+                for (int j = 0; j < EPN / 32; ++j)
+#pragma unroll
+                    for (int r = 0; r < 16; ++r)
+                        ep[(i * 32 + (r & 3) + 8 * (r >> 2) + 4 * (lane >> 5)) * EP_LD + j * 32 + (lane & 31)] = acc[i][h * (EPN / 32) + j][r];
+        }
         if constexpr (AMAX) {
             typedef float f4_t __attribute__((ext_vector_type(4)));
             if (lane < WM) {
@@ -501,6 +527,17 @@
     }
 }
 
+template <int BM, int BN, int WGM, int WGN, bool SPLIT, bool CONV, bool AMAX>
+__global__ __launch_bounds__(WGM* WGN * 64) void gemm_ps_kernel(GemmPsArgs p, int tiles_n, int tiles_total, int tiles_per_xcd,
+                                                                 uint32_t a_bytes, uint32_t w_bytes) {
+    gemm_ps_body<BM, BN, WGM, WGN, SPLIT, CONV, AMAX, false>(p, tiles_n, tiles_total, tiles_per_xcd, a_bytes, w_bytes);
+}
+template <int BM, int BN, int WGM, int WGN>
+__global__ __launch_bounds__(WGM* WGN * 64) void gemm_ps_glu_kernel(GemmPsArgs p, int tiles_n, int tiles_total, int tiles_per_xcd,
+                                                                     uint32_t a_bytes, uint32_t w_bytes) {
+    gemm_ps_body<BM, BN, WGM, WGN, true, false, false, true>(p, tiles_n, tiles_total, tiles_per_xcd, a_bytes, w_bytes);
+}
+
 template <int BM, int BN, int WGM, int WGN>
 void launch_ps_cfg(const GemmPsArgs& a, hipStream_t s) {
     const int tiles_m = cdiv(a.M, BM), tiles_n = cdiv(a.N, BN);
@@ -509,12 +546,15 @@
     char name[64];
     snprintf(name, sizeof(name), "gemm_%dx%d_presplit", BM, BN);
     prof::Scope scope(name, 2.0 * a.M * (double)a.N * a.K,
-                      4.0 * a.M * (double)a.K + 2.0 * a.N * (double)a.K + (a.amax ? 8.0 * a.M * (double)a.amax_ld : 4.0 * a.M * (double)a.N * (a.res ? 2.0 : 1.0)), s);
+                      4.0 * a.M * (double)a.K + 2.0 * a.N * (double)a.K + (a.amax ? 8.0 * a.M * (double)a.amax_ld : a.glu ? 2.0 * a.M * (double)a.N : 4.0 * a.M * (double)a.N * (a.res ? 2.0 : 1.0)), s);
     const dim3 grid(tiles_per_xcd * 8), block(WGM * WGN * 64);
     const uint32_t ab = (uint32_t)((int64_t)a.M * a.lda * 2), wb = (uint32_t)((int64_t)a.N * a.ldw * 2);
     const auto launch = [&](auto kernel) { hipLaunchKernelGGL(kernel, grid, block, 0, s, a, tiles_n, tiles_total, tiles_per_xcd, ab, wb); };
     const bool conv = a.conv_taps > 0;
-    if (a.amax) launch(gemm_ps_kernel<BM, BN, WGM, WGN, true, false, true>);
+    if (a.glu) {
+        if constexpr (BN >= 128) launch(gemm_ps_glu_kernel<BM, BN, WGM, WGN>);
+        else SC_CHECK(false, "presplit gemm: no GLU epilogue on the %d x %d tile", BM, BN);
+    } else if (a.amax) launch(gemm_ps_kernel<BM, BN, WGM, WGN, true, false, true>);
     else if (a.split && conv) launch(gemm_ps_kernel<BM, BN, WGM, WGN, true, true, false>);
     else if (a.split) launch(gemm_ps_kernel<BM, BN, WGM, WGN, true, false, false>);
     else if (conv) launch(gemm_ps_kernel<BM, BN, WGM, WGN, false, true, false>);
@@ -558,10 +598,34 @@
         SC_CHECK(a.amax_ld == gemm_presplit_amax_chunks(a.M, a.N), "presplit gemm: amax_ld=%d, this shape produces %d partial results per row",
                  a.amax_ld, gemm_presplit_amax_chunks(a.M, a.N));
     }
-    const int tile = ps_tile(a.M, a.N);
+    if (a.glu) {
+        SC_CHECK(a.split && a.conv_taps == 0 && !a.amax && a.C && !a.Ch && !a.res && !a.row_valid && a.act == ACT_NONE && a.alpha == 1.0f,
+                 "presplit gemm: the GLU epilogue takes a plain split product into C (no planes / residual / activation / alpha)");
+        SC_CHECK(a.N % 64 == 0 && a.ldc % 4 == 0 && a.ldc >= a.N / 2 && (a.glu_tile == 0 || a.glu_tile == 128 || a.glu_tile == 256),
+                 "presplit gemm: GLU epilogue with N=%d ldc=%lld tile=%d", a.N, (long long)a.ldc, a.glu_tile);
+    }
+    const int tile = a.glu ? (a.glu_tile ? a.glu_tile : std::max(ps_tile(a.M, a.N), 128)) : ps_tile(a.M, a.N);
     if (tile == 256) launch_ps_cfg<256, 256, 4, 2>(a, s);
     else if (tile == 128) launch_ps_cfg<128, 128, 2, 2>(a, s);
     else launch_ps_cfg<64, 64, 2, 2>(a, s);
+    SC_LAUNCH_CHECK();
+}
+
+bool gemm_presplit_glu_pays(int M, int N) { return ps_tile(M, N) >= 128; }
+
+namespace {
+__global__ __launch_bounds__(128) void glu_row_order_kernel(const __half* __restrict__ w, int64_t ldw, __half* __restrict__ out, int C, int k8) {
+    const int r = blockIdx.x;
+    const int src = (r >> 6) * 32 + (r & 31) + ((r & 32) ? C : 0);
+    const uint4* s = reinterpret_cast<const uint4*>(w + (int64_t)src * ldw);
+    uint4* d = reinterpret_cast<uint4*>(out + (int64_t)r * ldw);
+    for (int i = threadIdx.x; i < k8; i += 128) d[i] = s[i];
+}
+}
+
+void launch_glu_row_order(const __half* w, int64_t ldw, __half* out, int C, int K, hipStream_t s) {
+    SC_CHECK(C > 0 && C % 32 == 0 && K % 8 == 0 && ldw % 8 == 0 && ldw >= K, "glu_row_order: C=%d K=%d ldw=%lld", C, K, (long long)ldw);
+    hipLaunchKernelGGL(glu_row_order_kernel, dim3(2 * C), dim3(128), 0, s, w, ldw, out, C, (int)(ldw / 8));
     SC_LAUNCH_CHECK();
 }
 
diff --git a/seamless_communication_amd/csrc/k_misc.hip b/seamless_communication_amd/csrc/k_misc.hip
--- a/seamless_communication_amd/csrc/k_misc.hip
+++ b/seamless_communication_amd/csrc/k_misc.hip
@@ -410,6 +410,7 @@
 void launch_split_f32(const float* x, __half* hi, __half* lo, int64_t n, hipStream_t s) {
     SC_CHECK(n % 4 == 0, "split_f32: n must be a multiple of 4");
     if (n <= 0) return;
+    prof::Scope scope("split_f32", 2.0 * n, 8.0 * n, s);
     hipLaunchKernelGGL(split_f32_kernel, dim3(grid_for(n / 4)), dim3(256), 0, s, x, hi, lo, n / 4);
     SC_LAUNCH_CHECK();
 }
diff --git a/seamless_communication_amd/csrc/k_norm.hip b/seamless_communication_amd/csrc/k_norm.hip
--- a/seamless_communication_amd/csrc/k_norm.hip
+++ b/seamless_communication_amd/csrc/k_norm.hip
@@ -172,6 +172,7 @@
                              const float* bb2, __half* yh, __half* yl, int64_t ldh, int rows, int C, hipStream_t s) {
     SC_CHECK(C % 4 == 0 && C <= 1024 && ldx % 4 == 0 && ldy % 4 == 0 && ldh % 4 == 0 && y && yh && yl, "layernorm2_split: C=%d", C);
     if (rows <= 0) return;
+    prof::Scope scope("layernorm2_split", 16.0 * rows * (double)C, rows * (double)C * (4.0 + 4.0 + 4.0), s);
     hipLaunchKernelGGL(layernorm2_kernel, dim3(cdiv(rows, 4)), dim3(256), 0, s, x, ldx, ga, ba, y, ldy, gb2, bb2, yh, yl, ldh, rows, C);
     SC_LAUNCH_CHECK();
 }
@@ -181,6 +182,7 @@
     SC_CHECK(C % 4 == 0 && ldx % 4 == 0 && ldh % 4 == 0 && C <= 4096 && yh && yl, "layernorm_split: C=%d ldx=%lld ldh=%lld", C,
              (long long)ldx, (long long)ldh);
     if (rows <= 0) return;
+    prof::Scope scope("layernorm_split", 8.0 * rows * (double)C, rows * (double)C * (4.0 + 4.0), s);
     dim3 grid(cdiv(rows, 4));
     float* none = nullptr;
     if (C <= 256) hipLaunchKernelGGL((layernorm_kernel<1>), grid, dim3(256), 0, s, x, ldx, gamma, beta, none, (int64_t)0, rows, C, act, lens, t_per_batch, yh, yl, ldh);
@@ -349,7 +351,7 @@
     SC_LAUNCH_CHECK();
 }
 
-template <int K, int TT>
+template <int K, int TT, bool GATED>
 __global__ __launch_bounds__(1024) void glu_dwconv_ln_kernel(const float* __restrict__ x, int64_t ldx, const float* __restrict__ w,
                                                              const float* __restrict__ gamma, const float* __restrict__ beta, int act,
                                                              __half* __restrict__ yh, __half* __restrict__ yl, int64_t ldh, int T, int C,
@@ -374,8 +376,12 @@
         float v = 0.f;
         if (t >= 0 && t < len) {
             const float a = xn[(int64_t)t * ldx + c];
-            const float b = xn[(int64_t)t * ldx + C + c];
-            v = a / (1.f + expf(-b));
+            if constexpr (GATED) {
+                v = a;
+            } else {
+                const float b = xn[(int64_t)t * ldx + C + c];
+                v = a / (1.f + expf(-b));
+            }
         }
         g[i] = v;
     }
@@ -385,7 +391,7 @@
         const int t = t_begin + i;
         const bool ok = t < t_end && t < len;
         ra[i] = ok ? xn[(int64_t)t * ldx + c] : 0.f;
-        rb[i] = ok ? xn[(int64_t)t * ldx + C + c] : 0.f;
+        rb[i] = (!GATED && ok) ? xn[(int64_t)t * ldx + C + c] : 0.f;
     }
     const int nv = C >> 2;
     int buf = 0;
@@ -393,14 +399,15 @@
 #pragma unroll
         for (int i = 0; i < TT; ++i) {
             const int t = tc + i;
-            g[K - 1 + i] = (t < t_end && t < len) ? ra[i] / (1.f + expf(-rb[i])) : 0.f;
+            if constexpr (GATED) g[K - 1 + i] = (t < t_end && t < len) ? ra[i] : 0.f;
+            else g[K - 1 + i] = (t < t_end && t < len) ? ra[i] / (1.f + expf(-rb[i])) : 0.f;
         }
 #pragma unroll
         for (int i = 0; i < TT; ++i) {
             const int t = tc + TT + i;
             const bool ok = t < t_end && t < len;
             ra[i] = ok ? xn[(int64_t)t * ldx + c] : 0.f;
-            rb[i] = ok ? xn[(int64_t)t * ldx + C + c] : 0.f;
+            rb[i] = (!GATED && ok) ? xn[(int64_t)t * ldx + C + c] : 0.f;
         }
 #pragma unroll
         for (int tt = 0; tt < TT; ++tt) {
@@ -464,7 +471,7 @@
 bool glu_dwconv_ln_supported(int C, int ksize) { return ksize == 31 && C % 64 == 0 && C >= 64 && C <= 1024; }
 
 void launch_glu_dwconv_ln(const float* x, int64_t ldx, const float* w, const float* gamma, const float* beta, int act, __half* yh,
-                          __half* yl, int64_t ldh, int nb, int T, int C, int ksize, const int* lens, hipStream_t s) {
+                          __half* yl, int64_t ldh, int nb, int T, int C, int ksize, const int* lens, hipStream_t s, bool gated) {
     SC_CHECK(glu_dwconv_ln_supported(C, ksize) && ldh % 4 == 0, "glu_dwconv_ln: C=%d k=%d ldh=%lld unsupported", C, ksize, (long long)ldh);
     if (nb <= 0 || T <= 0) return;
     constexpr int TT = 8;
@@ -472,9 +479,13 @@
     const int range = cdiv(cdiv(T, ranges), TT) * TT;
     ranges = cdiv(T, range);
     const double rows = (double)nb * T;
-    prof::Scope scope("glu_dwconv_ln", 2.0 * rows * C * ksize, rows * C * (8.0 + 4.0), s);
-    hipLaunchKernelGGL((glu_dwconv_ln_kernel<31, TT>), dim3(ranges, nb), dim3(C), 0, s, x, ldx, w, gamma, beta, act, yh, yl, ldh, T, C, lens,
-                       range);
+    prof::Scope scope("glu_dwconv_ln", 2.0 * rows * C * ksize, rows * C * ((gated ? 4.0 : 8.0) + 4.0), s);
+    if (gated)
+        hipLaunchKernelGGL((glu_dwconv_ln_kernel<31, TT, true>), dim3(ranges, nb), dim3(C), 0, s, x, ldx, w, gamma, beta, act, yh, yl, ldh, T, C,
+                           lens, range);
+    else
+        hipLaunchKernelGGL((glu_dwconv_ln_kernel<31, TT, false>), dim3(ranges, nb), dim3(C), 0, s, x, ldx, w, gamma, beta, act, yh, yl, ldh, T, C,
+                           lens, range);
     SC_LAUNCH_CHECK();
 }
 
diff --git a/seamless_communication_amd/csrc/kernels.h b/seamless_communication_amd/csrc/kernels.h
--- a/seamless_communication_amd/csrc/kernels.h
+++ b/seamless_communication_amd/csrc/kernels.h
@@ -103,8 +103,11 @@
     const int2* row_pos = nullptr;
     float2* amax = nullptr;
     int amax_ld = 0;
+    int glu = 0, glu_tile = 0;
 };
 void launch_gemm_presplit(const GemmPsArgs& a, hipStream_t s);
+void launch_glu_row_order(const __half* w, int64_t ldw, __half* out, int C, int K, hipStream_t s);
+bool gemm_presplit_glu_pays(int M, int N);
 int gemm_presplit_amax_chunks(int M, int N);
 void launch_amax_finish(const float2* part, int ld, int rows, int* out_idx, hipStream_t s);
 
@@ -370,7 +373,7 @@
 
 bool glu_dwconv_ln_supported(int C, int ksize);
 void launch_glu_dwconv_ln(const float* x, int64_t ldx, const float* w, const float* gamma, const float* beta, int act, __half* yh,
-                          __half* yl, int64_t ldh, int nb, int T, int C, int ksize, const int* lens, hipStream_t s);
+                          __half* yl, int64_t ldh, int nb, int T, int C, int ksize, const int* lens, hipStream_t s, bool gated = false);
 void launch_glu_dwconv(const float* x, int64_t ldx, const float* w, float* y, int64_t ldy, int nb, int T,
                        int C, int ksize, const int* lens, hipStream_t s, int left = -1, const float* bn_scale = nullptr,
                        const float* bn_shift = nullptr);
diff --git a/seamless_communication_amd/csrc/model.h b/seamless_communication_amd/csrc/model.h
--- a/seamless_communication_amd/csrc/model.h
+++ b/seamless_communication_amd/csrc/model.h
@@ -90,6 +90,7 @@
 struct ConformerLayer {
     LNorm ffn1_ln, attn_ln, conv_ln, conv_inner_ln, ffn2_ln, final_ln;
     Linear ffn1_in, ffn1_out, ffn2_in, ffn2_out, qkv, attn_out, pw1, pw2;
+    Linear pw1_glu;
     const float* rel_k = nullptr;
     const float* dw = nullptr;
     Linear r_proj;
diff --git a/seamless_communication_amd/csrc/model_encoder.hip b/seamless_communication_amd/csrc/model_encoder.hip
--- a/seamless_communication_amd/csrc/model_encoder.hip
+++ b/seamless_communication_amd/csrc/model_encoder.hip
@@ -161,8 +161,9 @@
     auto ln_split = [&](const float* src, const LNorm& L, int act) {
         launch_layernorm_split(src, L.dim, L.g, L.b, hs_hi, hs_lo, L.dim, rows, L.dim, act, nullptr, 1, m.stream);
     };
+    static const bool single = knob::value("SC_SPLIT_MODE", 0) == 1;
     auto ps = [&](const __half* ah, const __half* al, const Linear& L, int act, float alpha, const float* res, float* C,
-                  __half* Ch, __half* Cl) {
+                  __half* Ch, __half* Cl, bool glu = false) {
         GemmPsArgs a;
         a.Ah = ah;
         a.Al = al;
@@ -173,7 +174,8 @@
         a.res = res;
         a.ldr = L.out;
         a.C = C;
-        a.ldc = L.out;
+        a.ldc = glu ? L.out / 2 : L.out;
+        a.glu = glu ? 1 : 0;
         a.Ch = Ch;
         a.Cl = Cl;
         a.ldcs = L.out;
@@ -182,7 +184,6 @@
         a.K = L.in;
         a.act = act;
         a.alpha = alpha;
-        static const bool single = knob::value("SC_SPLIT_MODE", 0) == 1;
         a.split = single ? 0 : 1;
         launch_gemm_presplit(a, m.stream);
     };
@@ -190,6 +191,9 @@
     static const bool fuse = knob::value("SC_ENC_FUSE", 1) != 0;
     const bool fuse_conv = fuse && glu_dwconv_ln_supported(M, c.depthwise_conv_kernel_size);
     const bool fuse_ln = fuse && M <= 1024;
+    const int glu_knob = knob::live("SC_ENC_GLU_EP", 1);
+    const bool glu_ep = fuse_conv && !single && M % 32 == 0 && glu_knob != 0 && (glu_knob >= 2 || gemm_presplit_glu_pays(rows, 2 * M)) &&
+                        c.enc_layers > 0 && m.enc[0].pw1_glu.w;
     bool ffn1_planes_ready = false;
     for (int li = 0; li < c.enc_layers; ++li) {
         const ConformerLayer& l = m.enc[li];
@@ -221,13 +225,19 @@
             }
             ps(as_hi, as_lo, l.attn_out, ACT_NONE, 1.f, x, x, nullptr, nullptr);
             ln_split(x, l.conv_ln, ACT_NONE);
-            ps(hs_hi, hs_lo, l.pw1, ACT_NONE, 1.f, nullptr, wide, nullptr, nullptr);
-            if (fuse_conv) {
-                launch_glu_dwconv_ln(wide, 2 * M, l.dw, l.conv_inner_ln.g, l.conv_inner_ln.b, ACT_SILU, hs_hi, hs_lo, M, n, S, M,
-                                     c.depthwise_conv_kernel_size, d_lens, m.stream);
+            if (glu_ep) {
+                ps(hs_hi, hs_lo, l.pw1_glu, ACT_NONE, 1.f, nullptr, wide, nullptr, nullptr, true);
+                launch_glu_dwconv_ln(wide, M, l.dw, l.conv_inner_ln.g, l.conv_inner_ln.b, ACT_SILU, hs_hi, hs_lo, M, n, S, M,
+                                     c.depthwise_conv_kernel_size, d_lens, m.stream, true);
             } else {
-                launch_glu_dwconv(wide, 2 * M, l.dw, att, M, n, S, M, c.depthwise_conv_kernel_size, d_lens, m.stream);
-                ln_split(att, l.conv_inner_ln, ACT_SILU);
+                ps(hs_hi, hs_lo, l.pw1, ACT_NONE, 1.f, nullptr, wide, nullptr, nullptr);
+                if (fuse_conv) {
+                    launch_glu_dwconv_ln(wide, 2 * M, l.dw, l.conv_inner_ln.g, l.conv_inner_ln.b, ACT_SILU, hs_hi, hs_lo, M, n, S, M,
+                                         c.depthwise_conv_kernel_size, d_lens, m.stream);
+                } else {
+                    launch_glu_dwconv(wide, 2 * M, l.dw, att, M, n, S, M, c.depthwise_conv_kernel_size, d_lens, m.stream);
+                    ln_split(att, l.conv_inner_ln, ACT_SILU);
+                }
             }
             ps(hs_hi, hs_lo, l.pw2, ACT_NONE, 1.f, x, x, nullptr, nullptr);
             ln_split(x, l.ffn2_ln, ACT_NONE);
diff --git a/seamless_communication_amd/csrc/model_load.hip b/seamless_communication_amd/csrc/model_load.hip
--- a/seamless_communication_amd/csrc/model_load.hip
+++ b/seamless_communication_amd/csrc/model_load.hip
@@ -371,6 +371,14 @@
         l.attn_out = L.lin(p + ".self_attn.output_proj", M, M);
         l.conv_ln = L.ln(p + ".conv_layer_norm", M);
         l.pw1 = L.lin_pw(p + ".conv.pointwise_conv1", 2 * M, M);
+        const bool glu_copy = c.enc_variant != 1 && knob::value("SC_PRESPLIT", 1) != 0 && knob::value("SC_ENC_FUSE", 1) != 0 &&
+                              knob::live("SC_ENC_GLU_EP", 1) != 0;
+        if (glu_copy) {
+            __half* d = static_cast<__half*>(L.dalloc((size_t)2 * M * l.pw1.ldw * 2));
+            launch_glu_row_order(l.pw1.w, l.pw1.ldw, d, M, M, m.stream);
+            l.pw1_glu = l.pw1;
+            l.pw1_glu.w = d;
+        }
         l.dw = L.f32(p + ".conv.depthwise_conv.weight", {M, 1, c.depthwise_conv_kernel_size});
         if (c.enc_variant == 1) {
             l.r_proj = L.lin(p + ".self_attn.sdpa.r_proj", M, M, false);
```

Result: no change. 337.9, median of 2 (+0.9%).
